# violetamenendez/zest-nerf

Hardware: AMD Instinct MI355X
Metric: rendered rays/sec (1024-ray x 128-sample batch per GPU) (higher is better)
Workload: dtype bf16; 1 GPU; nsff_static_1024x128; rays_per_gpu=1024, samples_per_ray=128, rays_total=1024, collective=none, ranks=1, backend=none

## Files before the change

### zest-nerf_amd/csrc/fused.cuh

```cuda
#pragma once
#include "mlp_engine.cuh"
#include "zest_sample_ops.cuh"

namespace zest {

constexpr int kMaxViews = 16;
constexpr int kCamStride = 24;

struct FusedNet {
    const float *bias;
    const uint4 *tiles;
    const float4 *vol;
    const float4 *imgs;
    const float *w2cs, *intr;
    int D, Hv, Wv, V, H, W;
    int head, v2;
};

struct FusedArgs {
    const float *ndc, *pts, *z, *dir;
    int R, S;
    FusedNet st, dy;
    float frame_idx;
    int white_bkgd;
    int bpr;
    float *partials;
    float *out;
    unsigned long long *stamps;
    int ray_ranges;
};

struct RayState {
    float Ts = 1.f, Tb = 1.f, Tf = 1.f;
    float s[5] = {0, 0, 0, 0, 0}, bl[5] = {0, 0, 0, 0, 0}, fg[4] = {0, 0, 0, 0};
    __device__ __forceinline__ void chain(const float *p, bool dyn) {
#pragma unroll
        for (int i = 0; i < 5; i++) s[i] += Ts * p[1 + i];
        Ts *= p[0];
        if (dyn) {
#pragma unroll
            for (int i = 0; i < 5; i++) bl[i] += Tb * p[7 + i];
            Tb *= p[6];
#pragma unroll
            for (int i = 0; i < 4; i++) fg[i] += Tf * p[13 + i];
            Tf *= p[12];
        }
    }
    __device__ __forceinline__ void emit(int white_bkgd, float *__restrict__ out_row) const {
        float4 *o = reinterpret_cast<float4 *>(out_row);
        const float bg = white_bkgd ? 1.0f - s[4] : 0.0f;
        o[0] = make_float4(s[0] + bg, s[1] + bg, s[2] + bg, s[3]);
        o[1] = make_float4(s[4], bl[0], bl[1], bl[2]);
        o[2] = make_float4(bl[3], fg[0], fg[1], fg[2]);
        float zero = 0.f;
        asm volatile("" : "+v"(zero));
        o[3] = make_float4(fg[3], bl[4], zero, zero);
    }
    __device__ __forceinline__ void save(float *c) const {
        c[0] = Ts, c[1] = Tb, c[2] = Tf;
#pragma unroll
        for (int i = 0; i < 5; i++) c[3 + i] = s[i], c[8 + i] = bl[i];
#pragma unroll
        for (int i = 0; i < 4; i++) c[13 + i] = fg[i];
    }
    __device__ __forceinline__ void load(const float *c) {
        Ts = c[0], Tb = c[1], Tf = c[2];
#pragma unroll
        for (int i = 0; i < 5; i++) s[i] = c[3 + i], bl[i] = c[8 + i];
#pragma unroll
        for (int i = 0; i < 4; i++) fg[i] = c[13 + i];
    }
};
constexpr int kCarryFloats = 20;

template <class Rec>
__device__ __forceinline__ void combine_ray(Rec rec, int bpr, bool dyn, int white_bkgd, float *__restrict__ out_row) {
    RayState st;
    for (int b = 0; b < bpr; b++) st.chain(rec(b), dyn);
    st.emit(white_bkgd, out_row);
}

template <int EP, int C, int L, int NK>
__device__ __forceinline__ void encode_pe_operand(const float (&x)[4], int grp, OpArr<NK, ep_parts(EP)> &op) {
    static_assert((L / 2) * C + 1 <= NK * 8 && L % 2 == 0, "position layout");
    const float quarter = (grp & 1) ? 0.25f : 0.0f;
    const float gscale = (grp & 2) ? 2.0f * 0.15915494309189535f : 0.15915494309189535f;
    const float gband = (grp & 2) ? 2.0f : 1.0f;
    float rev[C];
#pragma unroll
    for (int c = 0; c < C; c++) rev[c] = x[c] * gscale;
    const float raw = grp == 0 ? x[0] : (grp == 1 ? x[1] : (grp == 2 ? x[2] : (C > 3 ? x[3] : 0.0f)));
#pragma unroll
    for (int t = 0; t < NK; t++) {
        float v[8];
#pragma unroll
        for (int e = 0; e < 8; e++) {
            const int m = 8 * t + e;
            if (m < (L / 2) * C) {
                if constexpr (EP == ZEST_PREC_F16X3) {
                    float sn, cs;
                    zest_sincos(x[m % C] * (gband * (float)(1 << (2 * (m / C)))), &sn, &cs);
                    v[e] = (grp & 1) ? cs : sn;
                } else {
                    const float r = fmaf(rev[m % C], (float)(1 << (2 * (m / C))), quarter);
                    v[e] = __builtin_amdgcn_sinf(__builtin_amdgcn_fractf(r));
                }
            } else if (m == (L / 2) * C) {
                v[e] = raw;
            } else {
                v[e] = 0.0f;
            }
        }
        store_tile<EP>(v, op, t);
    }
}

__device__ __forceinline__ float4 zest_color_tap_fast(const float4 *__restrict__ img, int H, int W,
                                                      const float *__restrict__ P, float px, float py, float pz) {
    const float4 r0 = *reinterpret_cast<const float4 *>(P), r1 = *reinterpret_cast<const float4 *>(P + 4),
                 r2 = *reinterpret_cast<const float4 *>(P + 8);
    const float qx = fmaf(pz, r0.z, fmaf(py, r0.y, fmaf(px, r0.x, r0.w)));
    const float qy = fmaf(pz, r1.z, fmaf(py, r1.y, fmaf(px, r1.x, r1.w)));
    const float qz = fmaf(pz, r2.z, fmaf(py, r2.y, fmaf(px, r2.x, r2.w)));
    const float rz = __builtin_amdgcn_rcpf(qz);
    float fx = qx * rz, fy = qy * rz;
    const float wm = (float)(W - 1), hm = (float)(H - 1);
    const float mask = (fx > 0.0f && fx < wm && fy > 0.0f && fy < hm) ? 1.0f : 0.0f;
    fx = fminf(fmaxf(fx, 0.0f), wm), fy = fminf(fmaxf(fy, 0.0f), hm);
    const float x0f = floorf(fx), y0f = floorf(fy);
    const float tx = fx - x0f, ty = fy - y0f;
    const int x0 = (int)x0f, y0 = (int)y0f;
    const int i00 = y0 * W + x0, dx = x0 + 1 < W ? 1 : 0, dy = y0 + 1 < H ? W : 0;
    const float4 a = img[i00], b = img[i00 + dx], d = img[i00 + dy], e = img[i00 + dy + dx];
    const float w00 = (1.0f - tx) * (1.0f - ty), w10 = tx * (1.0f - ty), w01 = (1.0f - tx) * ty, w11 = tx * ty;
    float4 o;
    o.x = fmaf(w11, e.x, fmaf(w01, d.x, fmaf(w10, b.x, w00 * a.x)));
    o.y = fmaf(w11, e.y, fmaf(w01, d.y, fmaf(w10, b.y, w00 * a.y)));
    o.z = fmaf(w11, e.z, fmaf(w01, d.z, fmaf(w10, b.z, w00 * a.z)));
    o.w = mask;
    return o;
}

template <int EP, int NK>
__device__ __forceinline__ void encode_feat_operand(const FusedNet &n, const float *cams_lds,
                                                    const float (&ndc)[4], const float (&pw)[3],
                                                    int grp, bool valid, OpArr<NK, ep_parts(EP)> &op) {
    float v[NK * 8];
#pragma unroll
    for (int i = 0; i < NK * 8; i++) v[i] = 0.0f;
    auto view_tap = [&](int view, float *dst) {
        const int vc = view < n.V ? view : n.V - 1;
        const float *cl = cams_lds + vc * kCamStride;
        float4 o;
        if constexpr (EP == ZEST_PREC_F16X3) {
            ZestCam cam;
#pragma unroll
            for (int i = 0; i < 3; i++) {
#pragma unroll
                for (int j = 0; j < 4; j++) cam.r[i][j] = cl[4 * i + j];
#pragma unroll
                for (int j = 0; j < 3; j++) cam.k[i][j] = cl[12 + 3 * i + j];
            }
            o = zest_color_tap(n.imgs + (size_t)vc * n.H * n.W, n.H, n.W, cam, pw[0], pw[1], pw[2]);
        } else {
            o = zest_color_tap_fast(n.imgs + vc * (n.H * n.W), n.H, n.W, cl, pw[0], pw[1], pw[2]);
        }
        const bool on = view < n.V;
        dst[0] = on ? o.x : 0.f, dst[1] = on ? o.y : 0.f, dst[2] = on ? o.z : 0.f, dst[3] = on ? o.w : 0.f;
    };
    const int rv = feat_volume_round(n.V);
    if (valid) {
        float vv[4] = {0.f, 0.f, 0.f, 0.f};
        if (grp < 2) {
            float fx = zest_unnorm(ndc[0], n.Wv), fy = zest_unnorm(ndc[1], n.Hv), fz = zest_unnorm(ndc[2], n.D);
            fx = fminf(fmaxf(fx, -2.0f), (float)n.Wv + 1.0f);
            fy = fminf(fmaxf(fy, -2.0f), (float)n.Hv + 1.0f);
            fz = fminf(fmaxf(fz, -2.0f), (float)n.D + 1.0f);
            const float x0f = floorf(fx), y0f = floorf(fy), z0f = floorf(fz);
            const float tx = fx - x0f, ty = fy - y0f, tz = fz - z0f;
            const int x0 = (int)x0f, y0 = (int)y0f, z0 = (int)z0f;
            float4 tap[8];
            float wgt[8];
#pragma unroll
            for (int c = 0; c < 8; c++) {
                const int dx = c & 1, dy = (c >> 1) & 1, dz = c >> 2;
                const int xi = x0 + dx, yi = y0 + dy, zi = z0 + dz;
                const bool ok = (unsigned)xi < (unsigned)n.Wv && (unsigned)yi < (unsigned)n.Hv &&
                                (unsigned)zi < (unsigned)n.D;
                const int xc = min(max(xi, 0), n.Wv - 1), yc = min(max(yi, 0), n.Hv - 1),
                          zc = min(max(zi, 0), n.D - 1);
                wgt[c] = ok ? (dx ? tx : 1.0f - tx) * (dy ? ty : 1.0f - ty) * (dz ? tz : 1.0f - tz) : 0.0f;
                tap[c] = n.vol[2 * ((yc * n.Wv + xc) * n.D + zc) + grp];
            }
#pragma unroll
            for (int c = 0; c < 8; c++) {
                vv[0] = fmaf(wgt[c], tap[c].x, vv[0]), vv[1] = fmaf(wgt[c], tap[c].y, vv[1]);
                vv[2] = fmaf(wgt[c], tap[c].z, vv[2]), vv[3] = fmaf(wgt[c], tap[c].w, vv[3]);
            }
        }
#pragma unroll
        for (int r = 0; r < 2 * NK; r++) {
            float *dst = v + 8 * (r >> 1) + 4 * (r & 1);
            if (r < rv) {
                view_tap(4 * r + grp, dst);
            } else if (r == rv) {
                if (n.V > 4 * rv) view_tap(grp >= 2 ? 4 * rv + grp - 2 : n.V, dst);
                if (grp < 2) dst[0] = vv[0], dst[1] = vv[1], dst[2] = vv[2], dst[3] = vv[3];
            }
        }
    }
#pragma unroll
    for (int t = 0; t < NK; t++) {
        float w8[8];
#pragma unroll
        for (int e = 0; e < 8; e++) w8[e] = v[8 * t + e];
        store_tile<EP>(w8, op, t);
    }
}

template <bool PROJ>
__device__ __forceinline__ void stage_cams(const FusedNet &n, float *lds) {
    if (!n.w2cs) return;
    const int nv = n.imgs ? n.V : 1;
    for (int i = threadIdx.x; i < nv * kCamStride; i += blockDim.x) {
        const int v = i / kCamStride, k = i % kCamStride;
        float val = 0.0f;
        if constexpr (PROJ) {
            if (k < 12 && n.intr) {
                const int row = k >> 2, col = k & 3;
                const float *K = n.intr + 9 * v + 3 * row, *Rt = n.w2cs + 16 * v + col;
                val = fmaf(K[2], Rt[8], fmaf(K[1], Rt[4], K[0] * Rt[0]));
            } else if (k >= 12) {
                val = n.w2cs[16 * v + (k - 12)];
            }
        } else {
            if (k < 12) val = n.w2cs[16 * v + k];
            else if (k < 21 && n.intr) val = n.intr[9 * v + (k - 12)];
        }
        lds[i] = val;
    }
}

#ifndef ZEST_FUSED_WAVES
#define ZEST_FUSED_WAVES 8
#endif
constexpr int kFusedWaves = ZEST_FUSED_WAVES;
constexpr int kPartialFloats = 20;
constexpr int fused_cb(int EP) { return EP == ZEST_PREC_F16X3 ? 1 : 2; }

struct BlockSamples {
    float x[4], pw[3], zz, dist;
    bool valid;
};

template <int BS>
__device__ __forceinline__ float block_sum(float v) {
    if constexpr (BS == 32) return lower_half_sum(v);
    v += dpp_f<0xB1>(0.f, v);
    v += dpp_f<0x4E>(0.f, v);
    v += dpp_f<0x141>(0.f, v);
    v += dpp_f<0x140>(0.f, v);
    return readlane_f<0>(v);
}
template <int BS>
__device__ __forceinline__ float block_excl_prod(float f, int c, float *total) {
    if constexpr (BS == 32) return lower_half_excl_prod(f, c, total);
    float v = f;
    v *= dpp_f<0x111>(1.f, v);
    v *= dpp_f<0x112>(1.f, v);
    v *= dpp_f<0x114>(1.f, v);
    v *= dpp_f<0x118>(1.f, v);
    *total = readlane_f<15>(v);
    const float ex = dpp_f<0x138>(1.f, v);
    return c == 0 ? 1.0f : ex;
}

#ifndef ZEST_FUSED_WG_PER_CU
#define ZEST_FUSED_WG_PER_CU 1
#endif
template <int EP, int NT_FEAT_S, bool DYN, int NT_FEAT_D, bool V2S = false>
__global__ __launch_bounds__(kFusedWaves * 64, kFusedWaves * ZEST_FUSED_WG_PER_CU / 4) void fused_blocks_kernel(FusedArgs a) {
    constexpr bool MOD_S = NT_FEAT_S > 0, MOD_D = NT_FEAT_D > 0;
    constexpr int NP = ep_parts(EP), CB = fused_cb(EP), BS = 16 * CB;
    if constexpr (EP == ZEST_PREC_F16) engine_fp16_overflow_clamp();
    constexpr int UNITS_S = stream_units(4, NT_FEAT_S, NP, true), UNITS_D = DYN ? stream_units(6, NT_FEAT_D, NP, true) : 0;
    using Ring = RingTiles<kFusedWaves, UNITS_S, UNITS_D>;
    constexpr bool FEATURELESS = !MOD_S && !MOD_D;
    constexpr int PF = (NP == 1 && FEATURELESS) ? kPrefetchLone : kPrefetch;
    constexpr bool CONT = NP == 1 || FEATURELESS;
    constexpr int kStBytes = DYN ? kFusedWaves * 32 * 24 : 0;
    constexpr int kGapBytes = 2 * kSlots * 4;
    __shared__ __attribute__((aligned(16))) char lds[kRingUnits * 1024 + 2 * kMaxViews * kCamStride * 4 +
                                                     kFusedWaves * 32 * 8 + kGapBytes +
                                                     kFusedWaves * kPartialFloats * 4 + kFusedWaves * 32 * 16 +
                                                     kStBytes + 2 * kCarryFloats * 4];
    static_assert(sizeof(lds) <= 163840, "LDS budget of one workgroup per CU");
    float *cams_s = reinterpret_cast<float *>(lds + kRingUnits * 1024), *cams_d = cams_s + kMaxViews * kCamStride;
    float2 *zd_lds = reinterpret_cast<float2 *>(cams_d + kMaxViews * kCamStride);
    constexpr bool PROJ = EP != ZEST_PREC_F16X3;
    stage_cams<PROJ>(a.st, cams_s);
    if (DYN) stage_cams<PROJ>(a.dy, cams_d);
    char *gap = reinterpret_cast<char *>(zd_lds + kFusedWaves * 32);
    float *rec_lds = reinterpret_cast<float *>(gap + kGapBytes);
    float4 *x_lds = reinterpret_cast<float4 *>(rec_lds + kFusedWaves * kPartialFloats);
    float2 *st_lds = reinterpret_cast<float2 *>(x_lds + kFusedWaves * 32);
    float *carry_lds = reinterpret_cast<float *>(reinterpret_cast<char *>(st_lds) + kStBytes);
    __syncthreads();

    const int lane0 = threadIdx.x & 63;
    const int wave = __builtin_amdgcn_readfirstlane(threadIdx.x >> 6);
    const Ring tiles{lds, (gptr_u4)a.st.tiles, (gptr_u4)a.dy.tiles, lane0, lane0 >> 4, wave,
                     (unsigned)(wave * Ring::kPieces * 64 + lane0) * 16u,
                     (unsigned)(uintptr_t)(__attribute__((address_space(3))) char *)lds +
                         (unsigned)wave * Ring::kPieces * 1024u};
    tiles.init_addr();
    tiles.prologue();

    const bool ranges = a.ray_ranges != 0;
    const int n_wg = (int)gridDim.x;
    const int wg = n_wg % 8 == 0 ? (int)(blockIdx.x % 8) * (n_wg / 8) + (int)(blockIdx.x / 8) : (int)blockIdx.x;
    int range_b0, range_nb;
    if (ranges) {
        range_b0 = (int)((long long)wg * a.R / n_wg) * a.bpr;
        range_nb = (int)((long long)(wg + 1) * a.R / n_wg) * a.bpr - range_b0;
    } else {
        const int n_blocks = a.R * a.bpr;
        const int share = ((n_blocks + kFusedWaves - 1) / kFusedWaves + n_wg - 1) / n_wg * kFusedWaves;
        range_b0 = wg * share, range_nb = min(share, n_blocks - range_b0);
    }
    auto block_of = [&](int pass) {
        const int lb = pass * kFusedWaves + wave;
        return __builtin_amdgcn_readfirstlane(lb < range_nb ? range_b0 + lb : -1);
    };
    auto fetch = [&](int g, int cb, int col, BlockSamples &b) {
        const int r = g >= 0 ? g / a.bpr : 0, s = (g >= 0 ? g % a.bpr : 0) * BS + 16 * cb + col;
        b.valid = g >= 0 && s < a.S;
        b.x[0] = b.x[1] = b.x[2] = 0.f, b.x[3] = a.frame_idx;
        b.pw[0] = b.pw[1] = b.pw[2] = 0.f, b.zz = 0.f, b.dist = 0.f;
        const float *dir = a.dir + 3 * r;
        if (b.valid) {
            const size_t m = (size_t)r * a.S + s;
            const float *zr = a.z + (size_t)r * a.S;
            b.x[0] = a.ndc[3 * m], b.x[1] = a.ndc[3 * m + 1], b.x[2] = a.ndc[3 * m + 2];
            if (a.pts) b.pw[0] = a.pts[3 * m], b.pw[1] = a.pts[3 * m + 1], b.pw[2] = a.pts[3 * m + 2];
            b.zz = zr[s];
            const float dnorm = sqrtf(dir[0] * dir[0] + dir[1] * dir[1] + dir[2] * dir[2]);
            b.dist = ((s + 1 < a.S) ? (zr[s + 1] - b.zz) : 1e10f) * dnorm;
        }
    };
    auto join = [](const f32x4 (&t)[CB], int i) {
        if constexpr (CB == 1) {
            return t[0][i];
        } else {
            const auto r = __builtin_amdgcn_permlane16_swap(__float_as_uint(t[0][i]), __float_as_uint(t[CB - 1][i]), false, false);
            return __uint_as_float(r[0]);
        }
    };
#ifdef ZEST_STAMPS
    unsigned long long st_enc = 0, st_eng = 0, st_comp = 0, st_n = 0;
    const unsigned long long st_t0 = __builtin_amdgcn_s_memtime(), st_r0 = __builtin_amdgcn_s_memrealtime();
#define ZEST_STAMP(var) do { const unsigned long long t_ = __builtin_amdgcn_s_memtime(); var += t_ - st_last; st_last = t_; } while (0)
#else
#define ZEST_STAMP(var) do {} while (0)
#endif
    for (int k = 0; k * kFusedWaves < range_nb; k++) {
        const int pass = k;
#ifdef ZEST_STAMPS
        unsigned long long st_last = __builtin_amdgcn_s_memtime();
        st_n++;
#endif
        const int g = block_of(pass);
        if (__builtin_expect(g < 0, 0)) {
            tiles.finish(0, UNITS_S + UNITS_D);
        } else {
        int lane = lane0;
        asm volatile("" : "+v"(lane));
        const int col = lane & 15, grp = lane >> 4, cbs = lane & (BS - 1);
        int unit = 0;
        f32x4 head_s[CB], rgb_s[CB], head_d[CB], rgb_d[CB];
        auto views_of = [&](const FusedNet &n, const float *cams) {
            return [&, cams](OpArr<1, NP> (&views)[CB]) {
                const float *dir = a.dir + 3 * (g >= 0 ? g / a.bpr : 0);
                float dv[4] = {0.f, 0.f, 0.f, 0.f};
                zest_view_dir(dir, n.w2cs ? cams + (PROJ ? 12 : 0) : nullptr, dv);
                encode_pe_operand<EP, 3, 4, 1>(dv, grp, views[0]);
#pragma unroll
                for (int cb = 1; cb < CB; cb++) views[cb] = views[0];
            };
        };
        OpArr<NT_FEAT_S / 2, NP> feat_s[CB];
#pragma unroll
        for (int cb = 0; cb < CB; cb++) {
            BlockSamples b;
            fetch(g, cb, col, b);
            if (grp == 0) {
                zd_lds[wave * 32 + 16 * cb + col] = make_float2(b.zz, b.valid ? b.dist : -1.0f);
                x_lds[wave * 32 + 16 * cb + col] = make_float4(b.x[0], b.x[1], b.x[2], 0.0f);
            }
            if constexpr (MOD_S) encode_feat_operand<EP, NT_FEAT_S / 2>(a.st, cams_s, b.x, b.pw, grp, b.valid, feat_s[cb]);
            if constexpr (DYN && NT_FEAT_S >= 4) __builtin_amdgcn_sched_barrier(0);
        }
        auto pts_static = [&](OpArr<2, NP> (&o)[CB]) __attribute__((always_inline)) {
#pragma unroll
            for (int cb = 0; cb < CB; cb++) {
                int at = wave * 32 + 16 * cb + col;
                asm volatile("" : "+v"(at));
                const float4 xv = x_lds[at];
                const float x4[4] = {xv.x, xv.y, xv.z, 0.0f};
                encode_pe_operand<EP, 3, 10, 2>(x4, grp, o[cb]);
            }
        };
        auto pts_dynamic = [&](OpArr<3, NP> (&o)[CB]) __attribute__((always_inline)) {
#pragma unroll
            for (int cb = 0; cb < CB; cb++) {
                int at = wave * 32 + 16 * cb + col;
                asm volatile("" : "+v"(at));
                const float4 xv = x_lds[at];
                const float x4[4] = {xv.x, xv.y, xv.z, a.frame_idx};
                encode_pe_operand<EP, 4, 10, 3>(x4, grp, o[cb]);
            }
        };
        ZEST_STAMP(st_enc);
        {
            OpArr<2, NP> pts_keep[CB];
            pts_static(pts_keep);
            auto pts_copy = [&](OpArr<2, NP> (&o)[CB]) __attribute__((always_inline)) {
#pragma unroll
                for (int cb = 0; cb < CB; cb++) o[cb] = pts_keep[cb];
            };
            engine_forward<EP, CB, 4, MOD_S, NT_FEAT_S, V2S, true, PF, CONT>(tiles, unit, pts_copy, feat_s,
                                                                             views_of(a.st, cams_s), head_s, rgb_s);
        }
        ZEST_STAMP(st_eng);
        float rec[kPartialFloats];
#pragma unroll
        for (int i = 0; i < kPartialFloats; i++) rec[i] = 0.f;
        float zz, dist, cr, cg, cb, al_s;
        bool valid;
        {
            const float2 zd = zd_lds[wave * 32 + cbs];
            zz = zd.x, dist = fmaxf(zd.y, 0.0f), valid = zd.y >= 0.0f;
            float sg = join(head_s, 0);
            cr = join(rgb_s, 0), cg = join(rgb_s, 1), cb = join(rgb_s, 2);
            if (V2S) {
                cr = zest_sigmoid(cr), cg = zest_sigmoid(cg), cb = zest_sigmoid(cb), sg = fmaxf(sg, 0.f);
            }
            cr = zest_sigmoid(cr), cg = zest_sigmoid(cg), cb = zest_sigmoid(cb);
            al_s = valid ? 1.0f - expf(-fmaxf(sg, 0.f) * dist) : 0.0f;
            float tot;
            const float w = al_s * block_excl_prod<BS>(1.0f - al_s + 1e-10f, cbs, &tot);
            rec[0] = tot;
            rec[1] = block_sum<BS>(w * cr), rec[2] = block_sum<BS>(w * cg), rec[3] = block_sum<BS>(w * cb);
            rec[4] = block_sum<BS>(w * zz), rec[5] = block_sum<BS>(w);
        }
        if (DYN) {
            const float blend_s = zest_sigmoid(join(head_s, 1));
            if (lane < BS) {
                st_lds[(wave * 3 + 0) * 32 + lane] = make_float2(cr, cg);
                st_lds[(wave * 3 + 1) * 32 + lane] = make_float2(cb, al_s);
                st_lds[(wave * 3 + 2) * 32 + lane] = make_float2(blend_s, 0.0f);
            }
            OpArr<NT_FEAT_D / 2, NP> feat_d[CB];
            if constexpr (MOD_D) {
#pragma unroll
                for (int cbi = 0; cbi < CB; cbi++) {
                    BlockSamples b;
                    fetch(g, cbi, col, b);
                    encode_feat_operand<EP, NT_FEAT_D / 2>(a.dy, cams_d, b.x, b.pw, grp, b.valid, feat_d[cbi]);
                }
            }
            ZEST_STAMP(st_comp);
            {
                OpArr<3, NP> pts_keep[CB];
                pts_dynamic(pts_keep);
                auto pts_copy = [&](OpArr<3, NP> (&o)[CB]) __attribute__((always_inline)) {
#pragma unroll
                    for (int cb = 0; cb < CB; cb++) o[cb] = pts_keep[cb];
                };
                engine_forward<EP, CB, 6, MOD_D, NT_FEAT_D, false, true, PF, CONT>(tiles, unit, pts_copy, feat_d,
                                                                                   views_of(a.dy, cams_d), head_d, rgb_d);
            }
            ZEST_STAMP(st_eng);
            const float2 s0 = st_lds[(wave * 3 + 0) * 32 + cbs], s1 = st_lds[(wave * 3 + 1) * 32 + cbs],
                         s2 = st_lds[(wave * 3 + 2) * 32 + cbs];
            cr = s0.x, cg = s0.y, cb = s1.x, al_s = s1.y;
            const float blend = s2.x;
            const float er = zest_sigmoid(join(rgb_d, 0)), eg = zest_sigmoid(join(rgb_d, 1)),
                        eb = zest_sigmoid(join(rgb_d, 2));
            const float sg_d = join(head_d, 0);
            const float a_fg = valid ? 1.0f - expf(-fmaxf(sg_d, 0.f) * dist) : 0.0f;
            const float a_d = a_fg * blend, a_st = al_s * (1.0f - blend);
            float tot_b, tot_f;
            const float Tb = block_excl_prod<BS>((1.0f - a_d) * (1.0f - a_st) + 1e-10f, cbs, &tot_b);
            const float wf = a_fg * block_excl_prod<BS>(1.0f - a_fg + 1e-10f, cbs, &tot_f);
            const float wd = Tb * a_d, ws = Tb * a_st;
            rec[6] = tot_b;
            rec[7] = block_sum<BS>(wd * er + ws * cr), rec[8] = block_sum<BS>(wd * eg + ws * cg);
            rec[9] = block_sum<BS>(wd * eb + ws * cb), rec[10] = block_sum<BS>((wd + ws) * zz);
            rec[11] = block_sum<BS>(wd);
            rec[12] = tot_f;
            rec[13] = block_sum<BS>(wf * er), rec[14] = block_sum<BS>(wf * eg), rec[15] = block_sum<BS>(wf * eb);
            rec[16] = block_sum<BS>(wf * zz);
        }
        if (lane == 0 && g >= 0) {
            float4 *o = ranges ? reinterpret_cast<float4 *>(rec_lds + wave * kPartialFloats)
                               : reinterpret_cast<float4 *>(a.partials + (size_t)g * kPartialFloats);
#pragma unroll
            for (int i = 0; i < (DYN ? 5 : 2); i++)
                o[i] = make_float4(rec[4 * i], rec[4 * i + 1], rec[4 * i + 2], rec[4 * i + 3]);
        }
        }
        if (ranges) {
            __syncthreads();
            const int rb = g >= 0 ? g % a.bpr : 0;
            if (lane0 == 0 && g >= 0 && (wave == 0 || rb == 0)) {
                RayState st;
                if (rb != 0) st.load(carry_lds + ((k + 1) & 1) * kCarryFloats);
                const int n = min(a.bpr - rb, kFusedWaves - wave);
                for (int b = 0; b < n; b++) st.chain(rec_lds + (wave + b) * kPartialFloats, DYN);
                if (rb + n == a.bpr) st.emit(a.white_bkgd, a.out + (size_t)(g / a.bpr) * 16);
                else st.save(carry_lds + (k & 1) * kCarryFloats);
            }
        }
        ZEST_STAMP(st_comp);
    }
    tiles.drain();
#ifdef ZEST_STAMPS
    if (a.stamps && lane0 == 0) {
        unsigned long long *o = a.stamps + (size_t)(blockIdx.x * kFusedWaves + wave) * 8;
        o[0] = __builtin_amdgcn_s_memtime() - st_t0, o[1] = st_enc, o[2] = st_eng, o[3] = st_comp;
        o[4] = tiles.t_wait, o[5] = tiles.t_issue, o[6] = __builtin_amdgcn_s_memrealtime() - st_r0,
        o[7] = st_n | (tiles.t_vm << 16);
    }
#endif
}

#define ZEST_FUSED_VARIANT(ptag, EP, tag, NTS, DYN, NTD, V2S) ZEST_FUSED_VARIANT_(ptag, EP, tag, NTS, DYN, NTD, V2S)
#define ZEST_FUSED_VARIANT_(ptag, EP, tag, NTS, DYN, NTD, V2S)                                   \
    int fused_launch_##ptag##_##tag(const FusedArgs &a, int blocks, hipStream_t stream) {        \
        hipLaunchKernelGGL((fused_blocks_kernel<EP, NTS, DYN, NTD, V2S>), dim3(blocks),          \
                           dim3(kFusedWaves * 64), 0, stream, a);                                \
        ZEST_RETURN_LAUNCH("zest_render_fused_fwd(" #ptag "_" #tag ")");                         \
    }                                                                                            \
    int fused_units_##ptag##_##tag(int which) {                                                  \
        return which == 0 ? stream_units(4, NTS, ep_parts(EP), true) : (DYN ? stream_units(6, NTD, ep_parts(EP), true) : 0); \
    }

#define ZEST_FUSED_DECL1(ptag, tag)                                                     \
    int fused_launch_##ptag##_##tag(const FusedArgs &a, int blocks, hipStream_t stream); \
    int fused_units_##ptag##_##tag(int which);
#define ZEST_FUSED_DECL(tag) ZEST_FUSED_DECL1(bf16, tag) ZEST_FUSED_DECL1(f16, tag) ZEST_FUSED_DECL1(x3, tag)
ZEST_FUSED_DECL(s0)
ZEST_FUSED_DECL(s2)
ZEST_FUSED_DECL(s4)
ZEST_FUSED_DECL(s0d0)
ZEST_FUSED_DECL(s2d0)
ZEST_FUSED_DECL(s4d0)
ZEST_FUSED_DECL(s2d2)
ZEST_FUSED_DECL(s4d2)
ZEST_FUSED_DECL(s2v)
ZEST_FUSED_DECL(s4v)

}
```

### zest-nerf_amd/csrc/fused.hip

```cpp
#include <string.h>
#include "fused.cuh"
#include "mlp_plan.h"

namespace zest {

__global__ void fused_combine_kernel(const float *__restrict__ partials, int R, int bpr, int dyn,
                                     int white_bkgd, float *__restrict__ out) {
    const int r = blockIdx.x * blockDim.x + threadIdx.x;
    if (r >= R) return;
    combine_ray([&](int b) { return partials + ((size_t)r * bpr + b) * kPartialFloats; }, bpr, dyn != 0,
                white_bkgd, out + (size_t)r * 16);
}

}

namespace {

bool fill_net(const zest_mlp_desc *d, const void *packed, const zest_view_set *vs, int pts_ch, int precision,
              zest::FusedNet *n, int *nt_feat, int *units, const char **err) {
    memset(n, 0, sizeof(*n));
    if (!d || !packed) return *err = "descriptor and packed weights are required", false;
    if (d->in_ch_pts != pts_ch) return *err = "unexpected in_ch_pts for this slot", false;
    if (d->net_type != 0 && d->net_type != 2) return *err = "net_type must be 0 ('v0') or 2 ('v2')", false;
    zest::MlpPlan plan;
    if (!zest::build_plan(*d, precision, zest::ORDER_ACC, &plan, err, false, true)) return false;
    n->bias = (const float *)((const char *)packed + plan.stream_off);
    n->tiles = (const uint4 *)((const char *)n->bias + plan.bias_bytes);
    n->head = d->head, n->v2 = d->net_type == 2;
    *nt_feat = d->use_feat ? plan.nt_feat : 0;
    *units = plan.n_tiles;
    if (((uintptr_t)packed & 15) != 0) return *err = "packed weights must be 16-byte aligned", false;
    if (vs) {
        n->w2cs = vs->w2cs, n->intr = vs->intrinsics;
        n->vol = (const float4 *)vs->vol_cl, n->imgs = (const float4 *)vs->imgs_cl;
        n->D = vs->D, n->Hv = vs->Hv, n->Wv = vs->Wv, n->V = vs->V, n->H = vs->H, n->W = vs->W;
    }
    if (d->use_feat) {
        if (!vs || !vs->vol_cl || !vs->imgs_cl || !vs->w2cs || !vs->intrinsics)
            return *err = "a net with features needs volume, images and cameras", false;
        if (vs->D < 1 || vs->Hv < 1 || vs->Wv < 1 || vs->H < 2 || vs->W < 2)
            return *err = "bad volume / image shape", false;
        if ((long long)vs->D * vs->Hv * vs->Wv >= (1LL << 30))
            return *err = "volume too large for the fused kernel's 32-bit voxel indices (2^30 voxels)", false;
        if (vs->V < 1 || vs->V > zest::kMaxViews || 8 + 4 * vs->V != d->in_ch_feat)
            return *err = "view count does not match in_ch_feat = 8 + 4V", false;
        if (((uintptr_t)vs->vol_cl | (uintptr_t)vs->imgs_cl) & 15)
            return *err = "volume / images must be 16-byte aligned", false;
    } else {
        n->vol = nullptr, n->imgs = nullptr;
    }
    return true;
}

}

#ifdef ZEST_STAMPS
constexpr size_t kStampBytes = 1024 * 8 * 8 * 8;
#else
constexpr size_t kStampBytes = 0;
#endif

static int g_pass_shape = 0;

extern "C" int zest_render_fused_set_passes(int shape) {
    ZEST_CHECK_ARG(shape >= 0 && shape <= 2,
                   "zest_render_fused_set_passes: shape must be 0 (auto), 1 (dense: equal block shares) or 2 (ray ranges)");
    g_pass_shape = shape;
    return 0;
}

extern "C" int zest_render_fused_pass_shape(int R, int S, int precision, int cus, int *ray_ranges, int *n_wg,
                                            int *rounds) {
    ZEST_CHECK_ARG(R >= 0 && S >= 1 && zest::prec_is_engine(precision) && ray_ranges,
                   "zest_render_fused_pass_shape: bad argument");
    if (cus <= 0) {
        int dev = 0;
        if (hipGetDevice(&dev) != hipSuccess ||
            hipDeviceGetAttribute(&cus, hipDeviceAttributeMultiprocessorCount, dev) != hipSuccess)
            cus = 256;
    }
    const int bs = 16 * zest::fused_cb(precision), bpr = (S + bs - 1) / bs;
    const int W = zest::kFusedWaves;
    const int P = zest_div_up((long long)R * bpr, W), G0 = P < cus ? P : cus;
    const int dense_rounds = G0 ? zest_div_up(P, G0) : 0, dense_wg = G0 ? zest_div_up(P, dense_rounds) : 0;
    const int n = R < cus ? R : cus;
    const int range_rounds = n ? zest_div_up((long long)zest_div_up(R, n) * bpr, W) : 0;
    int take = range_rounds <= dense_rounds ? 1 : 0;
    if (g_pass_shape == 1) take = 0;
    if (g_pass_shape == 2) take = 1;
    *ray_ranges = take;
    if (n_wg) *n_wg = take ? n : dense_wg;
    if (rounds) *rounds = take ? range_rounds : dense_rounds;
    return 0;
}

extern "C" size_t zest_render_fused_workspace(int R, int S) {
    if (R <= 0 || S <= 0) return 16 + kStampBytes;
    return (size_t)R * ((S + 15) / 16) * zest::kPartialFloats * sizeof(float) + kStampBytes;
}

extern "C" int zest_render_fused_fwd(const float *ndc, const float *pts, const float *z,
                                     const float *rays_dir, int R, int S,
                                     const zest_mlp_desc *desc_static, const void *packed_static,
                                     const zest_view_set *views_static,
                                     const zest_mlp_desc *desc_dynamic, const void *packed_dynamic,
                                     const zest_view_set *views_dynamic, float frame_idx,
                                     int precision, int white_bkgd, void *workspace, float *out,
                                     void *stream) {
    if (R == 0) return 0;
    ZEST_CHECK_ARG(ndc && z && rays_dir && out && workspace,
                   "zest_render_fused_fwd: ndc, z, rays_dir, workspace, out required");
    ZEST_CHECK_ARG(((uintptr_t)workspace & 15) == 0, "zest_render_fused_fwd: workspace must be 16-byte aligned");
    ZEST_CHECK_ARG(R >= 0 && S >= 1, "zest_render_fused_fwd: bad shape R=%d S=%d", R, S);
    ZEST_CHECK_ARG(zest::prec_is_engine(precision),
                   "zest_render_fused_fwd: precision must be ZEST_PREC_BF16, _F16 or _F16X3 (the exact-product "
                   "fp32 kernel exists per operator only: zest_mlp_fwd)");
    ZEST_CHECK_ARG(((uintptr_t)out & 15) == 0, "zest_render_fused_fwd: out must be 16-byte aligned");
    zest::FusedArgs a;
    memset(&a, 0, sizeof(a));
    a.ndc = ndc, a.pts = pts, a.z = z, a.dir = rays_dir, a.R = R, a.S = S;
    a.frame_idx = frame_idx, a.white_bkgd = white_bkgd, a.out = out;
    const int bs = 16 * zest::fused_cb(precision);
    a.bpr = (S + bs - 1) / bs, a.partials = (float *)workspace;
#ifdef ZEST_STAMPS
    a.stamps = (unsigned long long *)((char *)workspace + zest_render_fused_workspace(R, S) - kStampBytes);
#endif
    const char *err = nullptr;
    int nts = 0, ntd = 0, units_s = 0, units_d = 0;
    ZEST_CHECK_ARG(fill_net(desc_static, packed_static, views_static, 63, precision, &a.st, &nts, &units_s, &err),
                   "zest_render_fused_fwd: static net: %s", err);
    const bool dyn = desc_dynamic != nullptr;
    if (dyn) {
        ZEST_CHECK_ARG(fill_net(desc_dynamic, packed_dynamic, views_dynamic, 84, precision, &a.dy, &ntd, &units_d, &err),
                       "zest_render_fused_fwd: dynamic net: %s", err);
        ZEST_CHECK_ARG(desc_static->head == ZEST_HEAD_BLEND && desc_dynamic->head == ZEST_HEAD_DYNAMIC,
                       "zest_render_fused_fwd: blending needs a static net with the blend head and "
                       "a dynamic net with the scene-flow heads");
    }
    ZEST_CHECK_ARG(pts || (!a.st.vol && !a.dy.vol), "zest_render_fused_fwd: pts required with features");
    if (R == 0) return 0;
    int dev = 0, cus = 256;
    if (hipGetDevice(&dev) != hipSuccess ||
        hipDeviceGetAttribute(&cus, hipDeviceAttributeMultiprocessorCount, dev) != hipSuccess)
        cus = 256;
    int blocks = 0;
    zest_render_fused_pass_shape(R, S, precision, cus, &a.ray_ranges, &blocks, nullptr);
    hipStream_t st = (hipStream_t)stream;
    const bool v2s = a.st.v2 != 0;
    ZEST_CHECK_ARG(!(v2s && (dyn || nts == 0)),
                   "zest_render_fused_fwd: a 'v2' net is rendered by the single-net kernels with features only");
    const int key = (v2s ? 1000 : 0) + (dyn ? 100 : 0) + nts * 10 + ntd;
    int rc = -1;
#define ZEST_CASE1(ptag, tag)                                                                    \
    ZEST_CHECK_ARG(zest::fused_units_##ptag##_##tag(0) == units_s && zest::fused_units_##ptag##_##tag(1) == units_d, \
                   "zest_render_fused_fwd: packed stream is %d+%d units, kernel expects %d+%d",  \
                   units_s, units_d, zest::fused_units_##ptag##_##tag(0), zest::fused_units_##ptag##_##tag(1)); \
    rc = zest::fused_launch_##ptag##_##tag(a, blocks, st);
#define ZEST_CASE(k, tag)                                                                        \
    case k:                                                                                      \
        if (precision == ZEST_PREC_BF16) { ZEST_CASE1(bf16, tag) }                               \
        else if (precision == ZEST_PREC_F16) { ZEST_CASE1(f16, tag) }                            \
        else { ZEST_CASE1(x3, tag) }                                                             \
        break;
    switch (key) {
        ZEST_CASE(0, s0)
        ZEST_CASE(20, s2)
        ZEST_CASE(40, s4)
        ZEST_CASE(100, s0d0)
        ZEST_CASE(120, s2d0)
        ZEST_CASE(140, s4d0)
        ZEST_CASE(122, s2d2)
        ZEST_CASE(142, s4d2)
        ZEST_CASE(1020, s2v)
        ZEST_CASE(1040, s4v)
        default:
            zest_set_error("zest_render_fused_fwd: no fused variant for %d static / %d dynamic feature "
                           "tiles%s", nts, ntd, dyn ? "" : " (static only)");
            return (int)hipErrorInvalidValue;
    }
#undef ZEST_CASE
#undef ZEST_CASE1
    if (rc != 0 || a.ray_ranges) return rc;
    hipLaunchKernelGGL(zest::fused_combine_kernel, dim3(zest_div_up(R, 128)), dim3(128), 0, st,
                       a.partials, R, a.bpr, dyn ? 1 : 0, white_bkgd, out);
    ZEST_RETURN_LAUNCH("zest_render_fused_fwd(combine)");
}
```

### zest-nerf_amd/csrc/mlp.hip

```cpp
#include <string.h>
#include <map>
#include <mutex>
#include <tuple>
#include "mlp_plan.h"
#include "zest_common.cuh"
#include "mlp_engine.cuh"

namespace {

using zest::MlpPlan;

struct DevPlan {
    MlpPlan plan;
    uint32_t *tile_src = nullptr, *bias_src = nullptr, *hdr_src = nullptr;
    uint8_t *unit_part = nullptr;
};

std::mutex g_mu;
std::map<std::tuple<int, int, int, int, int, int, int, int, int, int, int, int>, DevPlan *> g_plans;

constexpr int kOrderBwd = 99;
constexpr int kOrderFold = 98;

DevPlan *get_plan(const zest_mlp_desc &d, int precision, int order, bool need_tables) {
    int dev = 0;
    if (hipGetDevice(&dev) != hipSuccess) dev = 0;
    std::lock_guard<std::mutex> lk(g_mu);
    auto key = std::make_tuple(d.in_ch_pts, d.use_feat ? d.in_ch_feat : 0, d.in_ch_views,
                               d.use_feat, d.net_type, d.head, precision, order, d.depth, d.width, d.skip_mask, dev);
    auto it = g_plans.find(key);
    DevPlan *dp = it == g_plans.end() ? nullptr : it->second;
    if (!dp) {
        dp = new DevPlan();
        const char *err = nullptr;
        const bool ok = order == kOrderBwd    ? zest::build_bwd_plan(d, &dp->plan, &err)
                        : order == kOrderFold ? zest::build_plan(d, precision, zest::ORDER_ACC, &dp->plan, &err, true, true)
                                              : zest::build_plan(d, precision, order, &dp->plan, &err);
        if (!ok) {
            zest_set_error("MLP shape not supported: %s", err);
            delete dp;
            return nullptr;
        }
        g_plans[key] = dp;
    }
    if (need_tables && !dp->tile_src) {
        const size_t nt = dp->plan.tile_src.size() * 4, nb = dp->plan.bias_src.size() * 4;
        const size_t nh = dp->plan.hdr_src.size() * 4, np = dp->plan.unit_part.size();
        hipError_t e = hipMalloc(&dp->tile_src, nt);
        if (e == hipSuccess) e = hipMalloc(&dp->unit_part, np ? np : 4);
        if (e == hipSuccess && np) e = hipMemcpy(dp->unit_part, dp->plan.unit_part.data(), np, hipMemcpyHostToDevice);
        if (e == hipSuccess) e = hipMalloc(&dp->bias_src, nb ? nb : 4);
        if (e == hipSuccess) e = hipMalloc(&dp->hdr_src, nh ? nh : 4);
        if (e == hipSuccess) e = hipMemcpy(dp->tile_src, dp->plan.tile_src.data(), nt, hipMemcpyHostToDevice);
        if (e == hipSuccess && nb) e = hipMemcpy(dp->bias_src, dp->plan.bias_src.data(), nb, hipMemcpyHostToDevice);
        if (e == hipSuccess && nh) e = hipMemcpy(dp->hdr_src, dp->plan.hdr_src.data(), nh, hipMemcpyHostToDevice);
        if (e != hipSuccess) {
            zest_set_error("zest_mlp_pack: uploading gather tables: %s", hipGetErrorString(e));
            dp->tile_src = nullptr;
            return nullptr;
        }
    }
    return dp;
}

inline int order_for(int precision) {
    return zest::prec_is_engine(precision) ? zest::ORDER_ACC : zest::ORDER_NATURAL;
}

struct ParamTable {
    const float *p[2 * zest::kParamSlots];
};

__global__ __launch_bounds__(zest::kW) void fold_view_kernel(const float *__restrict__ wv, const float *__restrict__ bv,
                                                             const float *__restrict__ wf, const float *__restrict__ bf,
                                                             int ld_v, float *__restrict__ wc, float *__restrict__ bc) {
    constexpr int W = zest::kW;
    const int r = blockIdx.x, c = threadIdx.x;
    if (r < W / 2) {
        double acc = 0.0;
        for (int k = 0; k < W; k++) acc += (double)wv[(size_t)r * ld_v + k] * (double)wf[(size_t)k * W + c];
        wc[(size_t)r * W + c] = (float)acc;
    } else if (c < W / 2) {
        double acc = 0.0;
        for (int k = 0; k < W; k++) acc += (double)wv[(size_t)c * ld_v + k] * (double)bf[k];
        bc[c] = (float)(acc + (double)bv[c]);
    } else {
        bc[c] = 0.0f;
    }
}
static_assert(zest::kFoldScratchBytes == zest::kFoldBiasOffset + (size_t)zest::kW * 4, "bc [W/2] and W/2 floats of padding");

template <int PREC>
__global__ void pack_kernel(ParamTable pt, const uint32_t *__restrict__ tile_src, size_t n_w,
                            const uint32_t *__restrict__ bias_src, size_t n_b,
                            const uint8_t *__restrict__ unit_part,
                            float *__restrict__ bias_out, void *__restrict__ w_out) {
    const size_t i = (size_t)blockIdx.x * blockDim.x + threadIdx.x;
    if (i < n_b) {
        const uint32_t s = bias_src[i];
        bias_out[i] = s == 0xFFFFFFFFu ? 0.0f : pt.p[2 * (s >> 24) + 1][s & 0xFFFFFF];
    }
    if (i < n_w) {
        const uint32_t s = tile_src[i];
        const float v = s == 0xFFFFFFFFu ? 0.0f : pt.p[2 * (s >> 24)][s & 0xFFFFFF];
        if (PREC == ZEST_PREC_BF16) {
            ((__hip_bfloat16 *)w_out)[i] = __float2bfloat16(v);
        } else if (PREC == ZEST_PREC_F16) {
            ((_Float16 *)w_out)[i] = (_Float16)v;
        } else if (PREC == ZEST_PREC_F16X3) {
            const _Float16 hi = (_Float16)v;
            ((_Float16 *)w_out)[i] = unit_part[i / 512] ? (_Float16)((v - (float)hi) * 2048.0f) : hi;
        } else {
            ((float *)w_out)[i] = v;
        }
    }
}

__global__ void pack_headers_kernel(ParamTable pt, const uint32_t *__restrict__ hdr_src, size_t n,
                                    char *__restrict__ w_out) {
    const size_t i = (size_t)blockIdx.x * blockDim.x + threadIdx.x;
    if (i >= n) return;
    const uint32_t s = hdr_src[i];
    if (s == 0xFFFFFFFFu) return;
    const size_t unit = i / 64, j = i % 64;
    ((float *)(w_out + unit * 1024))[j] = pt.p[2 * (s >> 24) + 1][s & 0xFFFFFF];
}

struct F32Op {
    int njb, nseg, kind0, nt0, kind1, nt1, mod, relu, tile_base, tiles_per_jb, bias_block;
    int src_h, dst;
};
struct F32Prog {
    F32Op op[zest::kNumOps];
    int n_ops, W;
    int P, F, Vw, C_in, C_out, nt_feat, net_v2, act_out, head;
    int rows_pts, rows_feat;
};

constexpr int kF32Samples = 32;

__global__ __launch_bounds__(256, 1) void mlp_f32_kernel(F32Prog pr, const float *__restrict__ bias,
                                                         const float4 *__restrict__ tiles,
                                                         const float *__restrict__ x, int M,
                                                         float *__restrict__ out) {
    extern __shared__ __attribute__((aligned(16))) float smem[];
    float *b_pts = smem;
    float *b_feat = b_pts + pr.rows_pts * 32;
    float *b_views = b_feat + pr.rows_feat * 32;
    float *b_h[2] = {b_views + 32 * 32, b_views + 32 * 32 + pr.W * 32};
    const int tid = threadIdx.x, lane = tid & 63, wave = tid >> 6;
    const int col = lane & 31, half = lane >> 5;
    const int n_in_rows = pr.rows_pts + pr.rows_feat + 32;

    for (int m0 = blockIdx.x * kF32Samples; m0 < M; m0 += gridDim.x * kF32Samples) {
        __syncthreads();
        for (int i = tid; i < n_in_rows * 32; i += 256) smem[i] = 0.0f;
        __syncthreads();
        const int nvalid = min(kF32Samples, M - m0);
        for (int i = tid; i < nvalid * pr.C_in; i += 256) {
            const int s = i / pr.C_in, c = i % pr.C_in;
            const float v = x[(size_t)m0 * pr.C_in + i];
            float *dst = c < pr.P ? b_pts + c * 32
                                  : (c < pr.P + pr.F ? b_feat + (c - pr.P) * 32
                                                     : b_views + (c - pr.P - pr.F) * 32);
            dst[s] = v;
        }
        __syncthreads();
#pragma unroll 1
        for (int o = 0; o < pr.n_ops; o++) {
            const F32Op op = pr.op[o];
            for (int jb = wave; jb < op.njb; jb += 4) {
                const float4 *tp = tiles + ((size_t)op.tile_base + (size_t)jb * op.tiles_per_jb) * 64 + lane;
                f32x16 acc, macc;
                {
                    const float *bb = bias + (size_t)(op.bias_block + jb) * 32 + half * 16;
#pragma unroll
                    for (int i = 0; i < 16; i++) acc[i] = bb[i];
                }
                if (op.mod) {
                    const float *mb = bias + (size_t)jb * 32 + half * 16;
#pragma unroll
                    for (int i = 0; i < 16; i++) macc[i] = mb[i];
                    for (int t = 0; t < pr.nt_feat; t++, tp += 64) {
                        const float4 a = *tp;
                        const float *bp = b_feat + (t * 8 + 4 * half) * 32 + col;
                        macc = __builtin_amdgcn_mfma_f32_32x32x2f32(a.x, bp[0], macc, 0, 0, 0);
                        macc = __builtin_amdgcn_mfma_f32_32x32x2f32(a.y, bp[32], macc, 0, 0, 0);
                        macc = __builtin_amdgcn_mfma_f32_32x32x2f32(a.z, bp[64], macc, 0, 0, 0);
                        macc = __builtin_amdgcn_mfma_f32_32x32x2f32(a.w, bp[96], macc, 0, 0, 0);
                    }
                }
                for (int sg = 0; sg < op.nseg; sg++) {
                    const int kind = sg ? op.kind1 : op.kind0, nt = sg ? op.nt1 : op.nt0;
                    const float *src = kind == zest::SEG_PTS ? b_pts
                                       : kind == zest::SEG_VIEWS ? b_views : b_h[op.src_h];
                    for (int t = 0; t < nt; t++, tp += 64) {
                        const float4 a = *tp;
                        const float *bp = src + (t * 8 + 4 * half) * 32 + col;
                        acc = __builtin_amdgcn_mfma_f32_32x32x2f32(a.x, bp[0], acc, 0, 0, 0);
                        acc = __builtin_amdgcn_mfma_f32_32x32x2f32(a.y, bp[32], acc, 0, 0, 0);
                        acc = __builtin_amdgcn_mfma_f32_32x32x2f32(a.z, bp[64], acc, 0, 0, 0);
                        acc = __builtin_amdgcn_mfma_f32_32x32x2f32(a.w, bp[96], acc, 0, 0, 0);
                    }
                }
#pragma unroll
                for (int i = 0; i < 16; i++) {
                    const int row = 32 * jb + (i & 3) + 8 * (i >> 2) + 4 * half;
                    float v = acc[i];
                    if (op.mod) v = pr.net_v2 ? v + macc[i] : v * macc[i];
                    if (op.relu) v = fmaxf(v, 0.0f);
                    if (op.dst < 2) {
                        b_h[op.dst][row * 32 + col] = v;
                    } else if (col < nvalid) {
                        float *orow = out + (size_t)(m0 + col) * pr.C_out;
                        if (o == pr.n_ops - 1) {
                            if (row < 3) orow[row] = pr.act_out ? zest_sigmoid(v) : v;
                        } else if (row == 0) {
                            orow[3] = pr.act_out ? fmaxf(v, 0.0f) : v;
                        } else if (3 + row < pr.C_out) {
                            const bool is_sf = pr.head == ZEST_HEAD_DYNAMIC && row <= 6;
                            orow[3 + row] = is_sf ? tanhf(v) : zest_sigmoid(v);
                        }
                    }
                }
            }
            __syncthreads();
        }
    }
}

F32Prog make_f32_prog(const MlpPlan &p) {
    F32Prog pr = {};
    const int D = p.shape.D, t = (D - 1) & 1;
    pr.n_ops = p.n_ops, pr.W = p.shape.W;
    for (int o = 0; o < p.n_ops; o++) {
        const zest::OpPlan &s = p.op[o];
        F32Op &d = pr.op[o];
        const int src_h = o < D ? (o + 1) & 1 : (o == D + 2 ? 1 - t : t);
        const int dst = o < D ? o & 1 : (o == D + 1 ? 1 - t : (o == D + 2 ? t : 2));
        d.njb = s.njb, d.nseg = s.nseg, d.kind0 = s.seg[0].kind, d.nt0 = s.seg[0].ntiles;
        d.kind1 = s.seg[1].kind, d.nt1 = s.seg[1].ntiles, d.mod = s.mod, d.relu = s.relu;
        d.tile_base = s.tile_base, d.tiles_per_jb = s.tiles_per_jb, d.bias_block = s.bias_block;
        d.src_h = src_h, d.dst = dst;
    }
    pr.P = p.desc.in_ch_pts, pr.F = p.desc.use_feat ? p.desc.in_ch_feat : 0, pr.Vw = p.desc.in_ch_views;
    pr.C_in = pr.P + pr.F + pr.Vw;
    pr.C_out = p.desc.head == ZEST_HEAD_NONE ? 4 : (p.desc.head == ZEST_HEAD_BLEND ? 5 : 12);
    pr.nt_feat = p.nt_feat, pr.net_v2 = p.desc.net_type >= 2, pr.act_out = p.desc.net_type == 2, pr.head = p.desc.head;
    pr.rows_pts = p.nt_pts * 8, pr.rows_feat = p.nt_feat * 8;
    return pr;
}

}

namespace zest {
size_t bwd_stream_bytes(const zest_mlp_desc &d) {
    DevPlan *dp = get_plan(d, ZEST_PREC_BF16, kOrderBwd, false);
    return dp ? dp->plan.bytes : 0;
}
int bwd_stream_units_of(const zest_mlp_desc &d) {
    DevPlan *dp = get_plan(d, ZEST_PREC_BF16, kOrderBwd, false);
    return dp ? dp->plan.tail_unit0 : -1;
}
int pack_bwd_stream(const zest_mlp_desc &d, const float *const *params, void *packed, hipStream_t stream) {
    DevPlan *dp = get_plan(d, ZEST_PREC_BF16, kOrderBwd, true);
    if (!dp) return (int)hipErrorInvalidValue;
    const MlpPlan &p = dp->plan;
    ParamTable pt = {};
    for (int i = 0; i < 2 * ZEST_P_COUNT; i++) pt.p[i] = params[i];
    const size_t n_w = p.tile_src.size(), n_h = p.hdr_src.size();
    hipLaunchKernelGGL(pack_kernel<ZEST_PREC_BF16>, dim3(zest_div_up(n_w, 256)), dim3(256), 0, stream, pt, dp->tile_src,
                       n_w, dp->bias_src, (size_t)0, dp->unit_part, (float *)packed, packed);
    hipLaunchKernelGGL(pack_headers_kernel, dim3(zest_div_up(n_h, 256)), dim3(256), 0, stream, pt, dp->hdr_src, n_h,
                       (char *)packed);
    ZEST_RETURN_LAUNCH("zest_mlp_train16_pack");
}
}

extern "C" size_t zest_mlp_packed_bytes(const zest_mlp_desc *desc, int precision) {
    if (!desc) return 0;
    if (zest::prec_is_engine(precision)) {
        DevPlan *df = get_plan(*desc, precision, kOrderFold, false);
        return df ? df->plan.stream_off + df->plan.bytes : 0;
    }
    DevPlan *dp = get_plan(*desc, precision, order_for(precision), false);
    return dp ? dp->plan.bytes : 0;
}

extern "C" int zest_mlp_pack(const zest_mlp_desc *desc, int precision, const float *const *params,
                             void *packed, void *stream) {
    ZEST_CHECK_ARG(desc && params && packed, "zest_mlp_pack: null argument");
    DevPlan *dp = get_plan(*desc, precision, order_for(precision), true);
    if (!dp) return (int)hipErrorInvalidValue;
    const MlpPlan &p = dp->plan;
    DevPlan *df = zest::prec_is_engine(precision) ? get_plan(*desc, precision, kOrderFold, true) : nullptr;
    if (zest::prec_is_engine(precision) && !df) return (int)hipErrorInvalidValue;
    ParamTable pt = {};
    for (int i = 0; i < 2 * ZEST_P_COUNT; i++) pt.p[i] = params[i];
    bool need[ZEST_P_COUNT] = {};
    for (int i = 0; i < p.shape.D; i++) need[i] = true;
    need[ZEST_P_PTS_BIAS] = desc->use_feat != 0;
    need[ZEST_P_VIEWS] = need[ZEST_P_FEATURE] = need[ZEST_P_ALPHA] = need[ZEST_P_RGB] = true;
    need[ZEST_P_HEAD0] = desc->head != ZEST_HEAD_NONE;
    need[ZEST_P_HEAD1] = desc->head == ZEST_HEAD_DYNAMIC;
    for (int i = 0; i < ZEST_P_COUNT; i++)
        ZEST_CHECK_ARG(!need[i] || (params[2 * i] && params[2 * i + 1]),
                       "zest_mlp_pack: parameter slot %d (weight and bias) is required", i);
    ZEST_CHECK_ARG(((uintptr_t)packed & 15) == 0, "zest_mlp_pack: packed must be 16-byte aligned");
    auto pack_stream = [&](const DevPlan *q, char *base) {
        const size_t n_w = q->plan.tile_src.size(), n_b = q->plan.bias_src.size();
        const size_t n = n_w > n_b ? n_w : n_b;
        void *w_out = base + q->plan.bias_bytes;
#define ZEST_PACK(PREC)                                                                            \
    hipLaunchKernelGGL(pack_kernel<PREC>, dim3(zest_div_up(n, 256)), dim3(256), 0, (hipStream_t)stream, \
                       pt, q->tile_src, n_w, q->bias_src, n_b, q->unit_part, (float *)base, w_out)
        if (zest::prec_is_engine(precision)) {
            if (precision == ZEST_PREC_BF16) ZEST_PACK(ZEST_PREC_BF16);
            else if (precision == ZEST_PREC_F16) ZEST_PACK(ZEST_PREC_F16);
            else ZEST_PACK(ZEST_PREC_F16X3);
            const size_t n_h = q->plan.hdr_src.size();
            if (n_h)
                hipLaunchKernelGGL(pack_headers_kernel, dim3(zest_div_up(n_h, 256)), dim3(256), 0,
                                   (hipStream_t)stream, pt, q->hdr_src, n_h, (char *)w_out);
        } else {
            ZEST_PACK(ZEST_PREC_F32);
        }
#undef ZEST_PACK
    };
    pack_stream(dp, (char *)packed);
    if (df) {
        float *wc = (float *)((char *)packed + zest::fold_scratch_offset(p.bytes));
        float *bc = (float *)((char *)wc + zest::kFoldBiasOffset);
        hipLaunchKernelGGL(fold_view_kernel, dim3(zest::kW / 2 + 1), dim3(zest::kW), 0, (hipStream_t)stream,
                           params[2 * ZEST_P_VIEWS], params[2 * ZEST_P_VIEWS + 1], params[2 * ZEST_P_FEATURE],
                           params[2 * ZEST_P_FEATURE + 1], zest::kW + desc->in_ch_views, wc, bc);
        pt.p[2 * zest::kFoldSlot] = wc, pt.p[2 * zest::kFoldSlot + 1] = bc;
        pack_stream(df, (char *)packed + df->plan.stream_off);
    }
    ZEST_RETURN_LAUNCH("zest_mlp_pack");
}

extern "C" int zest_mlp_fwd(const zest_mlp_desc *desc, int precision, const void *packed,
                            const float *x, int M, float *out, void *stream) {
    if (M == 0) return 0;
    ZEST_CHECK_ARG(desc && packed && x && out, "zest_mlp_fwd: null argument");
    ZEST_CHECK_ARG(M >= 0, "zest_mlp_fwd: M=%d", M);
    DevPlan *dp = get_plan(*desc, precision, zest::prec_is_engine(precision) ? kOrderFold : order_for(precision), false);
    if (!dp) return (int)hipErrorInvalidValue;
    if (M == 0) return 0;
    const MlpPlan &p = dp->plan;
    const float *bias = (const float *)((const char *)packed + p.stream_off);
    const void *tiles = (const char *)bias + p.bias_bytes;
    if (precision == ZEST_PREC_F32) {
        const F32Prog pr = make_f32_prog(p);
        const size_t lds = (size_t)(pr.rows_pts + pr.rows_feat + 32 + 2 * pr.W) * 32 * sizeof(float);
        const int blocks = zest_div_up(M, kF32Samples);
        hipLaunchKernelGGL(mlp_f32_kernel, dim3(blocks < 4096 ? blocks : 4096), dim3(256), lds,
                           (hipStream_t)stream, pr, bias, (const float4 *)tiles, x, M, out);
        ZEST_RETURN_LAUNCH("zest_mlp_fwd(f32)");
    }
    return zest::mlp_engine_launch(p, tiles, x, M, out, (hipStream_t)stream);
}
```

### zest-nerf_amd/csrc/mlp_engine.cuh

```cuda
#pragma once
#include <hip/hip_bf16.h>
#include "mlp_plan.h"
#include "zest_common.cuh"

typedef __attribute__((ext_vector_type(16))) float f32x16;
typedef __attribute__((ext_vector_type(4))) float f32x4;
typedef __attribute__((ext_vector_type(8))) short bf16x8;
typedef __attribute__((ext_vector_type(4))) float v4f;
typedef __attribute__((ext_vector_type(4))) unsigned v4u;
typedef const __attribute__((address_space(1))) v4u *gptr_u4;

namespace zest {

constexpr int stream_units_raw(int nt_pts, int nt_feat, int parts = 1, bool fold = false) {
    const int mod = nt_feat * parts, P = nt_pts * parts, H = 16 * parts;
    return 8 * (1 + mod + P) + 6 * 8 * (1 + mod + H) + 8 * (1 + mod + P + H)
           + (1 + H) + (fold ? 0 : 8 * (1 + H)) + 4 * (1 + H + 2 * parts) + (1 + H / 2);
}
constexpr int stream_units(int nt_pts, int nt_feat, int parts = 1, bool fold = false) {
    return (stream_units_raw(nt_pts, nt_feat, parts, fold) + kStreamAlign - 1) / kStreamAlign * kStreamAlign;
}
static_assert(stream_units_raw(4, 0) == 1262 && stream_units_raw(4, 0, 1, true) == 1126 &&
              stream_units(4, 0, 1, true) == 9 * kStreamAlign, "unit counts of the headline net (DESIGN.md 3.1)");

#ifndef ZEST_CHUNK
#define ZEST_CHUNK 16
#define ZEST_SLOTS 8
#define ZEST_AHEAD 4
#endif
constexpr int kChunk = ZEST_CHUNK, kSlots = ZEST_SLOTS, kRingUnits = kChunk * kSlots, kAhead = ZEST_AHEAD;
static_assert(kStreamAlign % kRingUnits == 0, "stream padding must be a multiple of the ring size");
static_assert(kSlots >= kAhead + 1, "a slot is refilled while the previous chunk may still be read");

#ifndef ZEST_ISSUERS
#define ZEST_ISSUERS 8
#endif
template <int NW, int UNITS_A, int UNITS_B>
struct RingTiles {
    static constexpr int kIssuers = ZEST_ISSUERS < NW ? ZEST_ISSUERS : NW;
    static constexpr int kPieces = kChunk / kIssuers;
    static constexpr int kChunksA = UNITS_A / kChunk, kChunks = (UNITS_A + UNITS_B) / kChunk;
    static_assert(kChunk % kIssuers == 0 && UNITS_A % kRingUnits == 0 && UNITS_B % kRingUnits == 0, "");
    char *ring;
    gptr_u4 src_a, src_b;
    int lane, grp, wave;
    unsigned voff;
    unsigned lds_wave_base;
#ifdef ZEST_STAMPS
    mutable unsigned long long t_wait = 0, t_issue = 0, t_vm = 0;
#endif

    __device__ __forceinline__ void issue(int chunk) const {
        if (kIssuers < NW && wave >= kIssuers) return;
        const int c = chunk % kChunks;
        unsigned off = (unsigned)((c < kChunksA ? c : c - kChunksA) * kChunk * 1024);
        asm volatile("" : "+s"(off));
        const __attribute__((address_space(1))) char *sb =
            (const __attribute__((address_space(1))) char *)(c < kChunksA ? src_a : src_b) + off;
        const unsigned dst = lds_wave_base + (c % kSlots) * kChunk * 1024;
        static_assert(kPieces == 1 || kPieces == 2 || kPieces == 4, "pieces per wave");
        if (kPieces == 1)
            asm volatile("s_mov_b32 m0, %2\n\ts_nop 0\n\tglobal_load_lds_dwordx4 %0, %1"
                         :: "v"(voff), "s"(sb), "s"(dst) : "memory", "m0");
        else if (kPieces == 2)
            asm volatile("s_mov_b32 m0, %2\n\ts_nop 0\n\tglobal_load_lds_dwordx4 %0, %1\n\t"
                         "global_load_lds_dwordx4 %0, %1 offset:1024"
                         :: "v"(voff), "s"(sb), "s"(dst) : "memory", "m0");
        else
            asm volatile("s_mov_b32 m0, %2\n\ts_nop 0\n\tglobal_load_lds_dwordx4 %0, %1\n\t"
                         "global_load_lds_dwordx4 %0, %1 offset:1024\n\t"
                         "global_load_lds_dwordx4 %0, %1 offset:2048\n\t"
                         "global_load_lds_dwordx4 %0, %1 offset:3072"
                         :: "v"(voff), "s"(sb), "s"(dst) : "memory", "m0");
    }
    __device__ __forceinline__ void prologue() const {
#pragma unroll
        for (int c = 0; c < kAhead; c++) issue(c);
    }
    __device__ __forceinline__ void enter_chunk(int chunk) const {
#ifdef ZEST_STAMPS
        const unsigned long long t0 = __builtin_amdgcn_s_memtime();
#endif
        asm volatile("s_waitcnt vmcnt(%0)" ::"i"((kAhead - 1) * kPieces) : "memory");
#ifdef ZEST_STAMPS
        t_vm += __builtin_amdgcn_s_memtime() - t0;
#endif
        __builtin_amdgcn_s_barrier();
        asm volatile("" ::: "memory");
#ifdef ZEST_STAMPS
        const unsigned long long t1 = __builtin_amdgcn_s_memtime();
#endif
        issue(chunk + kAhead);
#ifdef ZEST_STAMPS
        t_wait += t1 - t0, t_issue += __builtin_amdgcn_s_memtime() - t1;
#endif
    }
    __device__ __forceinline__ void touch(int unit) const {
        if (unit % kChunk == 0) enter_chunk(unit / kChunk);
    }
    mutable unsigned rd_lo = 0, rd_hi = 0, rb_lo = 0, rb_hi = 0;
    __device__ __forceinline__ void init_addr() const {
        const unsigned base = (unsigned)(uintptr_t)(__attribute__((address_space(3))) char *)ring;
        rd_lo = base + lane * 16, rd_hi = rd_lo + 65536, rb_lo = base + grp * 16, rb_hi = rb_lo + 65536;
        asm volatile("" : "+v"(rd_lo), "+v"(rd_hi), "+v"(rb_lo), "+v"(rb_hi));
    }
    static_assert(kRingUnits <= 128, "two 64 KiB windows");
    template <class T>
    static __device__ __forceinline__ const __attribute__((address_space(3))) T *lds_at(unsigned addr) {
        return (const __attribute__((address_space(3))) T *)(uintptr_t)addr;
    }
    __device__ __forceinline__ bf16x8 load(int unit) const {
        touch(unit);
        const int r = unit % kRingUnits;
        const v4u v = *lds_at<v4u>((r < 64 ? rd_lo : rd_hi) + (r % 64) * 1024);
        return *reinterpret_cast<const bf16x8 *>(&v);
    }
    __device__ __forceinline__ f32x4 load_bias(int unit, int which, int rt) const {
        if (which == 0 && rt == 0) touch(unit);
        const int r = unit % kRingUnits;
        return *lds_at<v4f>((r < 64 ? rb_lo : rb_hi) + (r % 64) * 1024 + which * 128 + rt * 64);
    }
    __device__ __forceinline__ void finish(int unit, int end) const {
#pragma unroll
        for (int u = (unit + kChunk - 1) / kChunk * kChunk; u < end; u += kChunk) enter_chunk(u / kChunk);
    }
    __device__ __forceinline__ void drain() const { asm volatile("s_waitcnt vmcnt(0)" ::: "memory"); }
};

constexpr int ep_parts(int EP) { return EP == ZEST_PREC_F16X3 ? 2 : 1; }
constexpr float kLoScale = 2048.0f, kLoUnscale = 1.0f / 2048.0f;

typedef __attribute__((ext_vector_type(2))) float f32x2_t;
typedef __attribute__((ext_vector_type(2))) __bf16 bf16x2_t;
typedef __attribute__((ext_vector_type(2))) _Float16 f16x2_t;
typedef __attribute__((ext_vector_type(8))) _Float16 f16x8_t;

template <int EP>
__device__ __forceinline__ unsigned pack_pair(float lo, float hi) {
    const f32x2_t f = {lo, hi};
    if constexpr (EP == ZEST_PREC_BF16) {
        const bf16x2_t r = __builtin_convertvector(f, bf16x2_t);
        return __builtin_bit_cast(unsigned, r);
    } else {
        const f16x2_t r = __builtin_convertvector(f, f16x2_t);
        return __builtin_bit_cast(unsigned, r);
    }
}
__device__ __forceinline__ unsigned pack_bf16(float lo, float hi) { return pack_pair<ZEST_PREC_BF16>(lo, hi); }
__device__ __forceinline__ unsigned short bf16_bits(float v) { return (unsigned short)(pack_bf16(v, 0.f) & 0xFFFFu); }

__device__ __forceinline__ void split_pair(float a, float b, unsigned &hi, unsigned &lo) {
    const f32x2_t f = {a, b};
    const f16x2_t h = __builtin_convertvector(f, f16x2_t);
    const f32x2_t back = __builtin_convertvector(h, f32x2_t);
    const f32x2_t rem = {(a - back[0]) * kLoScale, (b - back[1]) * kLoScale};
    const f16x2_t l = __builtin_convertvector(rem, f16x2_t);
    hi = __builtin_bit_cast(unsigned, h), lo = __builtin_bit_cast(unsigned, l);
}

template <int EP>
__device__ __forceinline__ f32x4 mfma16(bf16x8 a, bf16x8 b, f32x4 c) {
    if constexpr (EP == ZEST_PREC_BF16)
        return __builtin_amdgcn_mfma_f32_16x16x32_bf16(a, b, c, 0, 0, 0);
    else
        return __builtin_amdgcn_mfma_f32_16x16x32_f16(__builtin_bit_cast(f16x8_t, a), __builtin_bit_cast(f16x8_t, b),
                                                      c, 0, 0, 0);
}

template <int EP>
__device__ __forceinline__ float relu1(float v) {
    return __builtin_amdgcn_fmed3f(v, 0.0f, EP == ZEST_PREC_BF16 ? 3.0e38f : 65504.0f);
}

template <int N, int NP = 1>
struct OpArr {
    bf16x8 t[NP][N > 0 ? N : 1];
};

template <int EP, int N>
__device__ __forceinline__ void store_tile(const float (&v)[8], OpArr<N, ep_parts(EP)> &op, int k) {
    if constexpr (EP == ZEST_PREC_F16X3) {
        uint4 h, l;
        split_pair(v[0], v[1], h.x, l.x), split_pair(v[2], v[3], h.y, l.y);
        split_pair(v[4], v[5], h.z, l.z), split_pair(v[6], v[7], h.w, l.w);
        op.t[0][k] = __builtin_bit_cast(bf16x8, h), op.t[1][k] = __builtin_bit_cast(bf16x8, l);
    } else {
        const uint4 q = make_uint4(pack_pair<EP>(v[0], v[1]), pack_pair<EP>(v[2], v[3]), pack_pair<EP>(v[4], v[5]),
                                   pack_pair<EP>(v[6], v[7]));
        op.t[0][k] = __builtin_bit_cast(bf16x8, q);
    }
}

typedef __attribute__((ext_vector_type(2))) short s16x2_t;
__device__ __forceinline__ unsigned relu_bf16x2(unsigned u) {
    const s16x2_t r = __builtin_elementwise_max(__builtin_bit_cast(s16x2_t, u), s16x2_t{0, 0});
    return __builtin_bit_cast(unsigned, r);
}
template <int EP, int N>
__device__ __forceinline__ void store_tile_relu16(const float (&v)[8], OpArr<N, 1> &op, int k) {
    const uint4 q = make_uint4(relu_bf16x2(pack_pair<EP>(v[0], v[1])), relu_bf16x2(pack_pair<EP>(v[2], v[3])),
                               relu_bf16x2(pack_pair<EP>(v[4], v[5])), relu_bf16x2(pack_pair<EP>(v[6], v[7])));
    op.t[0][k] = __builtin_bit_cast(bf16x8, q);
}
__device__ __forceinline__ void engine_fp16_overflow_clamp() {
    __builtin_amdgcn_s_setreg((0 << 11) | (23 << 6) | 1, 1);
}

#ifdef ZEST_PREFETCH
constexpr int kPrefetch = ZEST_PREFETCH, kPrefetchLone = ZEST_PREFETCH;
#else
constexpr int kPrefetch = 3, kPrefetchLone = 6;
#endif

template <int NP, int PF>
struct RowBlockPre {
    f32x4 bias[2], mbias[2];
    bf16x8 win[PF][NP];
};

struct NoSink {
    __device__ __forceinline__ void operator()(int, int, int, const float (&)[8]) const {}
};

template <int EP, int CB, int NJB, int NKA, int NKB, bool MOD, int NKF, bool RELU, int MODE, bool V2, int PF, bool CONT,
          class Tiles, class Sink = NoSink>
__device__ __forceinline__ void engine_layer(const Tiles &tiles, int &unit,
                                             const OpArr<NKA, ep_parts(EP)> (&opa)[CB],
                                             const OpArr<NKB, ep_parts(EP)> (&opb)[CB],
                                             const OpArr<NKF, ep_parts(EP)> (&opf)[CB],
                                             OpArr<8, ep_parts(EP)> (&out)[CB], f32x4 (&keep)[CB],
                                             int sink_id = 0, const Sink &sink = Sink()) {
    constexpr int NP = ep_parts(EP);
    constexpr bool X3 = EP == ZEST_PREC_F16X3;
    constexpr int NM = MOD ? 2 * NKF : 0, T = NM + 2 * (NKA + NKB);
    static_assert(T >= 1, "empty layer");
    constexpr bool kPackedRelu = RELU && MODE == 0 && EP != ZEST_PREC_F16X3 && __is_same(Sink, NoSink);
    constexpr int P = PF < T ? PF : T;
    auto preload_header = [&](RowBlockPre<NP, PF> &p, int u0) {
#pragma unroll
        for (int rt = 0; rt < 2; rt++) {
            p.bias[rt] = tiles.load_bias(u0, 0, rt);
            if (MOD) p.mbias[rt] = tiles.load_bias(u0, 1, rt);
        }
    };
    auto preload_tile = [&](RowBlockPre<NP, PF> &p, int u0, int k) {
#pragma unroll
        for (int pt = 0; pt < NP; pt++) p.win[k][pt] = tiles.load(u0 + 1 + NP * k + pt);
    };
    auto preload = [&](RowBlockPre<NP, PF> &p, int u0) {
        preload_header(p, u0);
#pragma unroll
        for (int k = 0; k < P; k++) preload_tile(p, u0, k);
    };
    RowBlockPre<NP, PF> pre;
    preload(pre, unit);
#pragma unroll
    for (int jb = 0; jb < NJB; jb++) {
        const int u0 = unit;
        f32x4 acc[2][CB], macc[2][CB], corr[2][CB], mcorr[2][CB];
        bf16x8 win[P][NP];
#pragma unroll
        for (int k = 0; k < P; k++)
#pragma unroll
            for (int pt = 0; pt < NP; pt++) win[k][pt] = pre.win[k][pt];
#pragma unroll
        for (int rt = 0; rt < 2; rt++)
#pragma unroll
            for (int cb = 0; cb < CB; cb++) {
                acc[rt][cb] = pre.bias[rt];
                if (MOD) macc[rt][cb] = pre.mbias[rt];
                if (X3) corr[rt][cb] = f32x4{0.f, 0.f, 0.f, 0.f}, mcorr[rt][cb] = f32x4{0.f, 0.f, 0.f, 0.f};
            }
#pragma unroll
        for (int k = 0; k < T; k++) {
            bf16x8 a[NP];
#pragma unroll
            for (int pt = 0; pt < NP; pt++) a[pt] = win[k % P][pt];
            const int rt = k % 2, kt = (k < NM ? k : k - NM) / 2;
#pragma unroll
            for (int cb = 0; cb < CB; cb++) {
                auto opnd = [&](int pt) -> bf16x8 {
                    if (k < NM) return opf[cb].t[pt][k < NM ? kt : 0];
                    if (kt < NKA) return opa[cb].t[pt][(k >= NM && kt < NKA) ? kt : 0];
                    return opb[cb].t[pt][(k >= NM && kt >= NKA) ? kt - NKA : 0];
                };
                if (k < NM) {
                    macc[rt][cb] = mfma16<EP>(a[0], opnd(0), macc[rt][cb]);
                    if constexpr (X3) {
                        mcorr[rt][cb] = mfma16<EP>(a[0], opnd(NP - 1), mcorr[rt][cb]);
                        mcorr[rt][cb] = mfma16<EP>(a[NP - 1], opnd(0), mcorr[rt][cb]);
                    }
                } else {
                    acc[rt][cb] = mfma16<EP>(a[0], opnd(0), acc[rt][cb]);
                    if constexpr (X3) {
                        corr[rt][cb] = mfma16<EP>(a[0], opnd(NP - 1), corr[rt][cb]);
                        corr[rt][cb] = mfma16<EP>(a[NP - 1], opnd(0), corr[rt][cb]);
                    }
                }
            }
            if (k + P < T) {
#pragma unroll
                for (int pt = 0; pt < NP; pt++) win[k % P][pt] = tiles.load(u0 + 1 + NP * (k + P) + pt);
            } else if (CONT && jb + 1 < NJB) {
                if (k + P == T) preload_header(pre, u0 + 1 + NP * T);
                preload_tile(pre, u0 + 1 + NP * T, k + P - T);
            }
        }
        unit = u0 + 1 + NP * T;
        if (!CONT && jb + 1 < NJB) preload(pre, unit);
#pragma unroll
        for (int cb = 0; cb < CB; cb++) {
            float v[8];
#pragma unroll
            for (int i = 0; i < 8; i++) {
                v[i] = acc[i >> 2][cb][i & 3];
                if (X3) v[i] = fmaf(corr[i >> 2][cb][i & 3], kLoUnscale, v[i]);
            }
            if (MOD) {
                float mv[8];
#pragma unroll
                for (int i = 0; i < 8; i++) {
                    mv[i] = macc[i >> 2][cb][i & 3];
                    if (X3) mv[i] = fmaf(mcorr[i >> 2][cb][i & 3], kLoUnscale, mv[i]);
                }
#pragma unroll
                for (int i = 0; i < 8; i++) v[i] = V2 ? v[i] + mv[i] : v[i] * mv[i];
            }
            if (RELU && !kPackedRelu) {
#pragma unroll
                for (int i = 0; i < 8; i++) v[i] = relu1<EP>(v[i]);
            }
            if (MODE == 0) {
                if constexpr (kPackedRelu) store_tile_relu16<EP>(v, out[cb], jb);
                else store_tile<EP>(v, out[cb], jb);
                sink(sink_id, jb, cb, v);
            } else if (jb == 0) {
                keep[cb] = f32x4{v[0], v[1], v[2], v[3]};
            }
        }
    }
}

template <int EP, int CB, int NU_PTS, bool MOD, int NU_FEAT, bool V2, bool FOLD = false, int PF = kPrefetch,
          bool CONT = false, class Tiles, class PtsFn, class ViewsFn, class Sink = NoSink>
__device__ __forceinline__ void engine_forward(const Tiles &tiles, int &unit, PtsFn pts_fn,
                                               const OpArr<NU_FEAT / 2, ep_parts(EP)> (&feat)[CB], ViewsFn views_fn,
                                               f32x4 (&head)[CB], f32x4 (&rgb)[CB], const Sink &sink = Sink()) {
    constexpr int KP = NU_PTS / 2, KF = NU_FEAT / 2, NP = ep_parts(EP);
    static_assert(NU_PTS % 2 == 0 && NU_FEAT % 2 == 0, "units per row block come in row-tile pairs");
    OpArr<8, NP> hA[CB], hB[CB];
    OpArr<0, NP> none[CB];
    f32x4 unused[CB];
    const int unit0 = unit;
    {
        OpArr<KP, NP> pts[CB];
        pts_fn(pts);
        engine_layer<EP, CB, 8, KP, 0, MOD, KF, true, 0, V2, PF, CONT>(tiles, unit, pts, none, feat, hA, unused, 0, sink);
    }
    engine_layer<EP, CB, 8, 8, 0, MOD, KF, true, 0, V2, PF, CONT>(tiles, unit, hA, none, feat, hB, unused, 1, sink);
    engine_layer<EP, CB, 8, 8, 0, MOD, KF, true, 0, V2, PF, CONT>(tiles, unit, hB, none, feat, hA, unused, 2, sink);
    engine_layer<EP, CB, 8, 8, 0, MOD, KF, true, 0, V2, PF, CONT>(tiles, unit, hA, none, feat, hB, unused, 3, sink);
    engine_layer<EP, CB, 8, 8, 0, MOD, KF, true, 0, V2, PF, CONT>(tiles, unit, hB, none, feat, hA, unused, 4, sink);
    {
        OpArr<KP, NP> pts[CB];
        pts_fn(pts);
        engine_layer<EP, CB, 8, KP, 8, MOD, KF, true, 0, V2, PF, CONT>(tiles, unit, pts, hA, feat, hB, unused, 5, sink);
    }
    engine_layer<EP, CB, 8, 8, 0, MOD, KF, true, 0, V2, PF, CONT>(tiles, unit, hB, none, feat, hA, unused, 6, sink);
    engine_layer<EP, CB, 8, 8, 0, MOD, KF, true, 0, V2, PF, CONT>(tiles, unit, hA, none, feat, hB, unused, 7, sink);
    engine_layer<EP, CB, 1, 8, 0, false, KF, false, 1, V2, PF, CONT>(tiles, unit, hB, none, feat, hA, head);
    if constexpr (!FOLD)
        engine_layer<EP, CB, 8, 8, 0, false, KF, false, 0, V2, PF, CONT>(tiles, unit, hB, none, feat, hA, unused, 8, sink);
    OpArr<8, NP> (&vin)[CB] = FOLD ? hB : hA, (&vout)[CB] = FOLD ? hA : hB;
    OpArr<1, NP> views[CB];
    views_fn(views);
    engine_layer<EP, CB, 4, 8, 1, false, KF, true, 0, V2, PF, CONT>(tiles, unit, vin, views, feat, vout, unused, 9, sink);
    OpArr<4, NP> h128[CB];
#pragma unroll
    for (int cb = 0; cb < CB; cb++)
#pragma unroll
        for (int pt = 0; pt < NP; pt++)
#pragma unroll
            for (int k = 0; k < 4; k++) h128[cb].t[pt][k] = vout[cb].t[pt][k];
    engine_layer<EP, CB, 1, 4, 0, false, KF, false, 1, V2, PF, CONT>(tiles, unit, h128, none, feat, vin, rgb);
    tiles.finish(unit, unit0 + stream_units(NU_PTS, MOD ? NU_FEAT : 0, NP, FOLD));
    unit = unit0 + stream_units(NU_PTS, MOD ? NU_FEAT : 0, NP, FOLD);
}

int mlp_engine_launch(const MlpPlan &p, const void *tiles, const float *x, int M, float *out,
                    hipStream_t stream);

}
```

### zest-nerf_amd/csrc/mlp_engine.hip

```cpp
#include "mlp_engine.cuh"
#include "mlp_train16.h"
#include "mlp_operands.cuh"

namespace zest {

constexpr int kMlpWaves = 8;
constexpr int mlp_cb(int EP) { return EP == ZEST_PREC_F16X3 ? 1 : 2; }

__device__ __forceinline__ void stash_store(uint4 *p, uint4 q) {
    __builtin_nontemporal_store(__builtin_bit_cast(v4u, q), reinterpret_cast<v4u *>(p));
}

template <int CB>
struct StashSink {
    uint4 *tiles;
    uint2 *masks;
    long long block;
    int lane;
    mutable unsigned lo[CB], hi[CB];
    __device__ __forceinline__ void operator()(int id, int jb, int cb, const float (&v)[8]) const {
        const int t = id < 8 ? 8 * id + jb : (id == 8 ? 64 + jb : 72 + jb);
        uint4 q = make_uint4(pack_bf16(v[0], v[1]), pack_bf16(v[2], v[3]), pack_bf16(v[4], v[5]), pack_bf16(v[6], v[7]));
        stash_store(&tiles[((block * kStashTiles + t) * CB + cb) * 64 + lane], q);
        if (id == 8) return;
        unsigned bits = 0;
#pragma unroll
        for (int i = 0; i < 8; i++) bits |= (v[i] > 0.0f ? 1u : 0u) << i;
        if (jb == 0) lo[cb] = 0, hi[cb] = 0;
        if (jb < 4) lo[cb] |= bits << (8 * jb);
        else hi[cb] |= bits << (8 * (jb - 4));
        const int last = id == 9 ? 3 : 7, mid = id == 9 ? 8 : id;
        if (jb == last) masks[((block * kStashMasks + mid) * CB + cb) * 64 + lane] = make_uint2(lo[cb], hi[cb]);
    }
};

template <int EP, int NT_PTS, bool MOD, int NT_FEAT, bool TRAIN = false, bool V2 = false>
__global__ __launch_bounds__(kMlpWaves * 64, kMlpWaves / 4) void mlp_engine_kernel(
    const uint4 *__restrict__ tiles_g, const float *__restrict__ x, int M, int P, int F, int C_in, int C_out, int head,
    int act_out, float *__restrict__ out, uint4 *__restrict__ stash_tiles = nullptr, uint2 *__restrict__ stash_masks = nullptr) {
    constexpr bool FOLD = !TRAIN;
    constexpr int NP = ep_parts(EP), CB = mlp_cb(EP), UNITS = stream_units(NT_PTS, MOD ? NT_FEAT : 0, NP, FOLD);
    using Ring = RingTiles<kMlpWaves, UNITS, 0>;
    if constexpr (EP == ZEST_PREC_F16) engine_fp16_overflow_clamp();
    __shared__ __attribute__((aligned(16))) char lds[kRingUnits * 1024 + 2 * kSlots * 4];
    const int lane = threadIdx.x & 63, col = lane & 15, grp = lane >> 4;
    const int wave = __builtin_amdgcn_readfirstlane(threadIdx.x >> 6);
    const Ring tiles{lds, (gptr_u4)tiles_g, (gptr_u4)tiles_g, lane, grp, wave,
                     (unsigned)(wave * Ring::kPieces * 64 + lane) * 16u,
                     (unsigned)(uintptr_t)(__attribute__((address_space(3))) char *)lds +
                         (unsigned)wave * Ring::kPieces * 1024u};
    tiles.init_addr();
    tiles.prologue();
    const int n_blocks = (M + 16 * CB - 1) / (16 * CB), n_pass = (n_blocks + kMlpWaves - 1) / kMlpWaves;
    for (int pass = blockIdx.x; pass < n_pass; pass += gridDim.x) {
        const long long m_base = ((long long)pass * kMlpWaves + wave) * (16 * CB);
        OpArr<NT_PTS / 2, NP> pts[CB];
        OpArr<NT_FEAT / 2, NP> feat[CB];
#pragma unroll
        for (int cb = 0; cb < CB; cb++) {
            const long long m = m_base + 16 * cb + col;
            const bool valid = m < M;
            const float *xrow = x + (size_t)(valid ? m : 0) * C_in;
            load_pe_operand<EP, NT_PTS == 4 ? 3 : 4, 10, NT_PTS / 2>(xrow, valid, grp, pts[cb]);
            if (MOD) load_feat_operand<EP, NT_FEAT / 2>(xrow + P, F, valid, grp, feat[cb]);
            if constexpr (TRAIN) {
                uint4 *st = stash_tiles + (((long long)pass * kMlpWaves + wave) * kStashTiles * CB + cb) * 64 + lane;
#pragma unroll
                for (int k = 0; k < NT_PTS / 2; k++) stash_store(&st[(size_t)(kStashPts + k) * CB * 64], __builtin_bit_cast(uint4, pts[cb].t[0][k]));
                if (MOD) {
#pragma unroll
                    for (int k = 0; k < NT_FEAT / 2; k++) stash_store(&st[(size_t)(kStashFeat + k) * CB * 64], __builtin_bit_cast(uint4, feat[cb].t[0][k]));
                }
            }
        }
        auto views_fn = [&](OpArr<1, NP> (&views)[CB]) {
#pragma unroll
            for (int cb = 0; cb < CB; cb++) {
                const long long m = m_base + 16 * cb + col;
                const bool valid = m < M;
                load_pe_operand<EP, 3, 4, 1>(x + (size_t)(valid ? m : 0) * C_in + P + F, valid, grp, views[cb]);
                if constexpr (TRAIN)
                    stash_store(&stash_tiles[((((long long)pass * kMlpWaves + wave) * kStashTiles + kStashViews) * CB + cb) * 64 + lane],
                                __builtin_bit_cast(uint4, views[cb].t[0][0]));
            }
        };
        f32x4 headt[CB], rgbt[CB];
        int unit = 0;
        auto pts_fn = [&](OpArr<NT_PTS / 2, NP> (&o)[CB]) {
#pragma unroll
            for (int cb = 0; cb < CB; cb++) o[cb] = pts[cb];
        };
        if constexpr (TRAIN) {
            const StashSink<CB> sink{stash_tiles, stash_masks, (long long)pass * kMlpWaves + wave, lane, {}, {}};
            engine_forward<EP, CB, NT_PTS, MOD, NT_FEAT, V2, false>(tiles, unit, pts_fn, feat, views_fn, headt, rgbt, sink);
        } else {
            engine_forward<EP, CB, NT_PTS, MOD, NT_FEAT, V2, true>(tiles, unit, pts_fn, feat, views_fn, headt, rgbt);
        }
#pragma unroll
        for (int cb = 0; cb < CB; cb++) {
            const long long m = m_base + 16 * cb + col;
            if (m >= M) continue;
            float *o = out + (size_t)m * C_out;
            if (grp == 0) {
                o[0] = act_out ? zest_sigmoid(rgbt[cb][0]) : rgbt[cb][0];
                o[1] = act_out ? zest_sigmoid(rgbt[cb][1]) : rgbt[cb][1];
                o[2] = act_out ? zest_sigmoid(rgbt[cb][2]) : rgbt[cb][2];
                o[3] = act_out ? fmaxf(headt[cb][0], 0.0f) : headt[cb][0];
                if (head == ZEST_HEAD_BLEND) o[4] = zest_sigmoid(headt[cb][1]);
                if (head == ZEST_HEAD_DYNAMIC)
                    o[4] = tanhf(headt[cb][1]), o[5] = tanhf(headt[cb][2]), o[6] = tanhf(headt[cb][3]);
            } else if (head == ZEST_HEAD_DYNAMIC && grp == 1) {
                o[7] = tanhf(headt[cb][0]), o[8] = tanhf(headt[cb][1]), o[9] = tanhf(headt[cb][2]);
                o[10] = zest_sigmoid(headt[cb][3]);
            } else if (head == ZEST_HEAD_DYNAMIC && grp == 2) {
                o[11] = zest_sigmoid(headt[cb][0]);
            }
        }
    }
    tiles.drain();
}

template <int EP, int NT_PTS, bool MOD, int NT_FEAT, bool TRAIN = false, bool V2 = false>
static int launch_one(const MlpPlan &p, const void *tiles, const float *x, int M,
                      float *out, hipStream_t stream, void *stash_tiles = nullptr, void *stash_masks = nullptr) {
    constexpr int units = stream_units(NT_PTS, MOD ? NT_FEAT : 0, ep_parts(EP), !TRAIN);
    if (p.n_tiles != units || (p.fold != 0) != !TRAIN) {
        zest_set_error("zest_mlp_fwd(engine): plan has %d stream units (fold %d), kernel expects %d (fold %d)", p.n_tiles,
                       p.fold, units, TRAIN ? 0 : 1);
        return (int)hipErrorInvalidValue;
    }
    const zest_mlp_desc &d = p.desc;
    const int F = d.use_feat ? d.in_ch_feat : 0;
    const int C_in = d.in_ch_pts + F + d.in_ch_views;
    const int C_out = d.head == ZEST_HEAD_NONE ? 4 : (d.head == ZEST_HEAD_BLEND ? 5 : 12);
    int dev = 0, cus = 256;
    if (hipGetDevice(&dev) != hipSuccess ||
        hipDeviceGetAttribute(&cus, hipDeviceAttributeMultiprocessorCount, dev) != hipSuccess)
        cus = 256;
    const int n_pass = zest_div_up(zest_div_up(M, 16 * mlp_cb(EP)), kMlpWaves);
    const int blocks = n_pass < cus ? n_pass : cus;
    if ((d.net_type >= 2) != V2) {
        zest_set_error("zest_mlp_fwd(engine): kernel / net_type mismatch");
        return (int)hipErrorInvalidValue;
    }
    hipLaunchKernelGGL((mlp_engine_kernel<EP, NT_PTS, MOD, NT_FEAT, TRAIN, V2>), dim3(blocks), dim3(kMlpWaves * 64), 0, stream,
                       (const uint4 *)tiles, x, M, d.in_ch_pts, F, C_in, C_out, d.head,
                       d.net_type == 2 ? 1 : 0, out, (uint4 *)stash_tiles, (uint2 *)stash_masks);
    ZEST_RETURN_LAUNCH(TRAIN ? "zest_mlp_train16_fwd" : "zest_mlp_fwd(engine)");
}

template <int EP>
static int launch_prec(const MlpPlan &p, const void *tiles, const float *x, int M, float *out, hipStream_t stream) {
    const bool mod = p.desc.use_feat != 0;
    const int key = p.nt_pts * 10 + (mod ? p.nt_feat : 0);
    if (p.desc.net_type >= 2) {
        switch (key) {
            case 42: return launch_one<EP, 4, true, 2, false, true>(p, tiles, x, M, out, stream);
            case 44: return launch_one<EP, 4, true, 4, false, true>(p, tiles, x, M, out, stream);
            case 62: return launch_one<EP, 6, true, 2, false, true>(p, tiles, x, M, out, stream);
            case 64: return launch_one<EP, 6, true, 4, false, true>(p, tiles, x, M, out, stream);
        }
        zest_set_error("zest_mlp_fwd(engine): no 'v2' kernel for %d point units / %d feature units per row block",
                       p.nt_pts, mod ? p.nt_feat : 0);
        return (int)hipErrorInvalidValue;
    }
    switch (key) {
        case 40: return launch_one<EP, 4, false, 0>(p, tiles, x, M, out, stream);
        case 42: return launch_one<EP, 4, true, 2>(p, tiles, x, M, out, stream);
        case 44: return launch_one<EP, 4, true, 4>(p, tiles, x, M, out, stream);
        case 60: return launch_one<EP, 6, false, 0>(p, tiles, x, M, out, stream);
        case 62: return launch_one<EP, 6, true, 2>(p, tiles, x, M, out, stream);
        case 64: return launch_one<EP, 6, true, 4>(p, tiles, x, M, out, stream);
    }
    zest_set_error("zest_mlp_fwd(engine): no kernel for %d point units / %d feature units per row "
                   "block (supported: 1..14 source views)", p.nt_pts, mod ? p.nt_feat : 0);
    return (int)hipErrorInvalidValue;
}

int mlp_engine_train_launch(const MlpPlan &p, const void *tiles, const float *x, int M, float *out, void *stash_tiles,
                            void *stash_masks, hipStream_t stream) {
    constexpr int EP = ZEST_PREC_BF16;
    const bool mod = p.desc.use_feat != 0;
    const int key = p.nt_pts * 10 + (mod ? p.nt_feat : 0);
    switch (key) {
        case 40: return launch_one<EP, 4, false, 0, true>(p, tiles, x, M, out, stream, stash_tiles, stash_masks);
        case 42: return launch_one<EP, 4, true, 2, true>(p, tiles, x, M, out, stream, stash_tiles, stash_masks);
        case 44: return launch_one<EP, 4, true, 4, true>(p, tiles, x, M, out, stream, stash_tiles, stash_masks);
        case 60: return launch_one<EP, 6, false, 0, true>(p, tiles, x, M, out, stream, stash_tiles, stash_masks);
        case 62: return launch_one<EP, 6, true, 2, true>(p, tiles, x, M, out, stream, stash_tiles, stash_masks);
        case 64: return launch_one<EP, 6, true, 4, true>(p, tiles, x, M, out, stream, stash_tiles, stash_masks);
    }
    zest_set_error("zest_mlp_train16_fwd: no kernel for %d point units / %d feature units per row block", p.nt_pts,
                   mod ? p.nt_feat : 0);
    return (int)hipErrorInvalidValue;
}

int mlp_engine_launch(const MlpPlan &p, const void *tiles, const float *x, int M, float *out,
                      hipStream_t stream) {
    switch (p.precision) {
        case ZEST_PREC_BF16: return launch_prec<ZEST_PREC_BF16>(p, tiles, x, M, out, stream);
        case ZEST_PREC_F16: return launch_prec<ZEST_PREC_F16>(p, tiles, x, M, out, stream);
        case ZEST_PREC_F16X3: return launch_prec<ZEST_PREC_F16X3>(p, tiles, x, M, out, stream);
    }
    zest_set_error("zest_mlp_fwd(engine): precision %d is not an engine operand type", p.precision);
    return (int)hipErrorInvalidValue;
}

}
```

### zest-nerf_amd/csrc/mlp_plan.h

```cpp
#pragma once
#include <stdint.h>
#include <vector>
#include "../../include/zest_render.h"

#ifdef __HIPCC__
#define ZEST_HD __host__ __device__
#else
#define ZEST_HD
#endif

namespace zest {

ZEST_HD inline int feat_volume_round(int V) { return V % 4 <= 2 ? V / 4 : V / 4 + 1; }
ZEST_HD inline int feat_quad_col(int q, int V) {
    const int r = 2 * (q >> 3) + (q & 1), g = (q & 7) >> 1, rv = feat_volume_round(V);
    if (r > rv) return -1;
    if (r == rv && g < 2) return 4 * g;
    const int view = r < rv ? 4 * r + g : 4 * rv + g - 2;
    return view < V ? 8 + 4 * view : -1;
}

constexpr int kW = 256;
constexpr int kNumOps = 12;
constexpr int kMaxSeg = 2;
constexpr int kStreamAlign = 128;

constexpr int kFoldSlot = ZEST_P_COUNT;
constexpr int kParamSlots = ZEST_P_COUNT + 1;
constexpr size_t kFoldBiasOffset = (size_t)(kW / 2) * kW * 4;
constexpr size_t kFoldScratchBytes = (kFoldBiasOffset + (size_t)(kW / 2) * 4 + 1023) / 1024 * 1024;
constexpr size_t fold_scratch_offset(size_t plain_bytes) { return plain_bytes; }
constexpr size_t infer_stream_offset(size_t plain_bytes) { return plain_bytes + kFoldScratchBytes; }

enum SlotOrder {
    ORDER_ACC = 0,
    ORDER_NATURAL = 1,
};

enum SegKind { SEG_PTS = 0, SEG_FEAT = 1, SEG_VIEWS = 2, SEG_H = 3 };

struct SegPlan {
    int kind;
    int ntiles;
};

struct OpPlan {
    int njb;
    int nseg;
    SegPlan seg[kMaxSeg];
    int mod;
    int relu;
    int tile_base;
    int tiles_per_jb;
    int bias_block;
};

struct MlpShape {
    int D, W, skip_mask;
    bool is_default;
};
bool mlp_shape(const zest_mlp_desc &d, MlpShape *s, const char **err);
void mlp_param_ld(const zest_mlp_desc &d, const MlpShape &s, int *ld);

struct MlpPlan {
    zest_mlp_desc desc;
    MlpShape shape;
    int n_ops;
    int precision, order;
    int spt;
    int ns_pts, ns_feat, ns_views;
    int nt_pts, nt_feat, nt_views, nt_h, nt_h128;
    int tail_unit0;
    int headers;
    int parts;
    int fold;
    size_t stream_off;
    int n_tiles, n_bias_blocks;
    size_t bias_bytes, bytes;
    OpPlan op[kNumOps];
    std::vector<int16_t> map_pts, map_feat, map_views;
    std::vector<uint32_t> tile_src, bias_src;
    std::vector<uint32_t> hdr_src;
    std::vector<uint8_t> unit_part;
};

inline bool prec_is_engine(int precision) {
    return precision == ZEST_PREC_BF16 || precision == ZEST_PREC_F16 || precision == ZEST_PREC_F16X3;
}

bool build_bwd_plan(const zest_mlp_desc &d, MlpPlan *out, const char **err);
constexpr int bwd_stream_units_raw(int nt_pts, int nt_feat) {
    const int kp = nt_pts / 2, mod = nt_feat;
    return 4 * (1 + 2 * 1)
           + 8 * (1 + 2 * 4)
           + 8 * (1 + mod + 2 * 9)
           + 6 * 8 * (1 + mod + 2 * 8)
           + kp * (1 + 2 * 8) + 8 * (1 + mod + 2 * 8)
           + kp * (1 + 2 * 8);
}
constexpr int bwd_stream_units(int nt_pts, int nt_feat) {
    return (bwd_stream_units_raw(nt_pts, nt_feat) + kStreamAlign - 1) / kStreamAlign * kStreamAlign;
}

struct DwJob {
    int32_t out_tile0, n_out_tiles;
    int32_t in_kind;
    int32_t in_tile0, n_in_tiles;
    int32_t ld, col0, want_bias;
    int32_t wg0, n_wg;
    int16_t out_slot[256], out_row[256];
    int16_t in_col[256];
};
constexpr int kGradTiles = 86;
constexpr int kDwStashPts = 76, kDwStashFeat = 79, kDwStashViews = 81;
int build_dw_jobs(const zest_mlp_desc &d, std::vector<DwJob> *jobs, const char **err);

bool build_plan(const zest_mlp_desc &d, int precision, int order, MlpPlan *out, const char **err,
                bool with_tables = true, bool fold = false);

}
```

### zest-nerf_amd/csrc/mlp_plan.hip

```cpp
#include "mlp_plan.h"
#include <string.h>

namespace zest {

namespace {

inline int round_up(int a, int b) { return (a + b - 1) / b * b; }

void pe_map_acc(int C, int L, int npos, std::vector<int16_t> &m) {
    m.assign((size_t)npos, -1);
    for (int pos = 0; pos < npos; pos++) {
        const int kt = pos / 32, g = (pos % 32) / 8, e = pos % 8, mm = 8 * kt + e;
        if (mm < (L / 2) * C) {
            const int band = 2 * (mm / C) + (g >> 1), coord = mm % C;
            m[pos] = (int16_t)(C + 2 * C * band + ((g & 1) ? C : 0) + coord);
        } else if (mm == (L / 2) * C) {
            m[pos] = (int16_t)(g < C ? g : -1);
        }
    }
}

void feat_map_acc(int V, int npos, std::vector<int16_t> &m) {
    m.assign((size_t)npos, -1);
    for (int pos = 0; pos < npos; pos++) {
        const int kt = pos / 32, g = (pos % 32) / 8, e = pos % 8, q = 8 * kt + 2 * g + (e >> 2), c = e & 3;
        const int col = feat_quad_col(q, V);
        if (col >= 0) m[pos] = (int16_t)(col + c);
    }
}

void natural_map(int width, int spt, int ntiles, std::vector<int16_t> &m) {
    m.assign((size_t)ntiles * spt * 2, -1);
    for (int t = 0; t < ntiles; t++)
        for (int j = 0; j < spt; j++)
            for (int h = 0; h < 2; h++) {
                const int f = t * 2 * spt + spt * h + j;
                m[2 * (t * spt + j) + h] = (int16_t)(f < width ? f : -1);
            }
}

inline int h_feature(int order, int spt, int slot, int half) {
    if (order == ORDER_ACC) {
        const int kt = slot / 32, g = (slot % 32) / 8, e = slot % 8;
        return 32 * kt + (e < 4 ? 4 * g + e : 16 + 4 * g + (e - 4));
    }
    const int t = slot / spt, j = slot % spt;
    return t * 2 * spt + spt * half + j;
}

struct RowSrc { int param, row; };

}

bool build_plan(const zest_mlp_desc &d, int precision, int order, MlpPlan *P, const char **err,
                bool with_tables, bool fold) {
    static const char *e_prec = "precision must be ZEST_PREC_F32, _BF16, _F16 or _F16X3";
    static const char *e_pts = "in_ch_pts must be 63 (xyz, L=10) or 84 (xyzt, L=10)";
    static const char *e_views = "in_ch_views must be 27 (L=4)";
    static const char *e_feat = "in_ch_feat must be 8 + 4V with 1 <= V <= 16 when use_feat is set";
    static const char *e_head = "bad head / net_type combination";
    if (precision != ZEST_PREC_F32 && !prec_is_engine(precision)) return *err = e_prec, false;
    if ((order == ORDER_ACC) != prec_is_engine(precision))
        return *err = "ORDER_ACC goes with the engine precisions, ORDER_NATURAL with fp32", false;
    if (fold && order != ORDER_ACC) return *err = "only the engine's stream (ORDER_ACC) has a folded form", false;
    if (d.in_ch_pts != 63 && d.in_ch_pts != 84) return *err = e_pts, false;
    if (d.in_ch_views != 27) return *err = e_views, false;
    const int F = d.use_feat ? d.in_ch_feat : 0;
    if (d.use_feat && (F < 12 || (F - 8) % 4 != 0 || F > 72)) return *err = e_feat, false;
    if (d.head < 0 || d.head > 2 || (d.net_type != 0 && d.net_type != 2 && d.net_type != 3) ||
        (d.net_type >= 2 && (d.head != 0 || !d.use_feat)))
        return *err = e_head, false;

    MlpShape sh;
    if (!mlp_shape(d, &sh, err)) return false;
    if (order == ORDER_ACC && !sh.is_default)
        return *err = "the MFMA engine covers depth 8 / width 256 / skips [4]; other shapes run in ZEST_PREC_F32", false;
    const int D = sh.D, Wd = sh.W;

    MlpPlan &p = *P;
    p.desc = d, p.precision = precision, p.order = order, p.shape = sh;
    p.n_ops = D + 4;
    p.spt = prec_is_engine(precision) ? 8 : 4;
    p.parts = precision == ZEST_PREC_F16X3 ? 2 : 1;
    p.fold = fold ? 1 : 0, p.stream_off = 0;
    const int spt = p.spt, C = d.in_ch_pts == 63 ? 3 : 4, V = d.use_feat ? (F - 8) / 4 : 0;
    if (order == ORDER_ACC) {
        p.ns_pts = 32 * ((5 * C + 1 + 7) / 8);
        p.ns_views = 32;
        p.ns_feat = d.use_feat ? round_up(4 * (2 + V), 32) : 0;
        pe_map_acc(C, 10, p.ns_pts, p.map_pts);
        pe_map_acc(3, 4, p.ns_views, p.map_views);
        if (d.use_feat) feat_map_acc(V, p.ns_feat, p.map_feat);
    } else {
        p.ns_pts = round_up(d.in_ch_pts, 2 * spt) / 2;
        p.ns_views = round_up(27, 2 * spt) / 2;
        p.ns_feat = d.use_feat ? round_up(F, 2 * spt) / 2 : 0;
        natural_map(d.in_ch_pts, spt, p.ns_pts / spt, p.map_pts);
        natural_map(27, spt, p.ns_views / spt, p.map_views);
        if (d.use_feat) natural_map(F, spt, p.ns_feat / spt, p.map_feat);
    }
    const int spu = order == ORDER_ACC ? 16 : spt;
    p.nt_pts = p.ns_pts / spu, p.nt_views = p.ns_views / spu, p.nt_feat = p.ns_feat / spu;
    p.nt_h = order == ORDER_ACC ? 16 : Wd / 2 / spt, p.nt_h128 = order == ORDER_ACC ? 8 : Wd / 4 / spt;

    p.headers = order == ORDER_ACC ? 1 : 0;
    memset(p.op, 0, sizeof(p.op));
    int tile = 0, bblk = d.use_feat ? Wd / 32 : 0;
    for (int o = 0; o < p.n_ops; o++) {
        OpPlan &op = p.op[o];
        op.njb = Wd / 32, op.nseg = 1, op.seg[0] = {SEG_H, p.nt_h};
        if (o < D) op.mod = d.use_feat ? 1 : 0, op.relu = 1;
        if (o == 0) op.seg[0] = {SEG_PTS, p.nt_pts};
        if (o > 0 && o < D && (sh.skip_mask >> (o - 1) & 1))
            op.nseg = 2, op.seg[0] = {SEG_PTS, p.nt_pts}, op.seg[1] = {SEG_H, p.nt_h};
        if (o == D) op.njb = 1;
        if (o == D + 1 && fold) op.njb = 0;
        if (o == D + 2) op.njb = Wd / 64, op.relu = 1, op.nseg = 2, op.seg[1] = {SEG_VIEWS, p.nt_views};
        if (o == D + 3) op.njb = 1, op.seg[0] = {SEG_H, p.nt_h128};
        op.tiles_per_jb = (op.mod ? p.nt_feat : 0) * p.parts + p.headers;
        for (int s = 0; s < op.nseg; s++) op.tiles_per_jb += op.seg[s].ntiles * p.parts;
        op.tile_base = tile, op.bias_block = bblk;
        tile += op.njb * op.tiles_per_jb, bblk += op.njb;
    }
    if (p.headers) tile = round_up(tile, kStreamAlign), bblk = 0;
    p.n_tiles = tile, p.n_bias_blocks = bblk;
    p.bias_bytes = (size_t)round_up(bblk * 128, 1024);
    p.bytes = p.bias_bytes + (size_t)tile * 1024;
    if (fold) {
        MlpPlan plain;
        if (!build_plan(d, precision, order, &plain, err, false, false)) return false;
        p.stream_off = infer_stream_offset(plain.bytes);
    }

    if (!with_tables) return true;
    int ld[ZEST_P_COUNT];
    mlp_param_ld(d, sh, ld);
    const uint32_t ZERO = 0xFFFFFFFFu;
    p.tile_src.assign((size_t)tile * 64 * spt, ZERO);
    p.bias_src.assign(p.bias_bytes / 4, ZERO);
    p.hdr_src.assign(p.headers ? (size_t)tile * 64 : 0, ZERO);
    p.unit_part.assign((size_t)tile, 0);

    auto row_src = [&](int o, int row) -> RowSrc {
        if (o < D) return {ZEST_P_PTS0 + o, row};
        if (o == D + 1) return {ZEST_P_FEATURE, row};
        if (o == D + 2) return {row < Wd / 2 ? (fold ? kFoldSlot : ZEST_P_VIEWS) : -1, row};
        if (o == D + 3) return {row < 3 ? ZEST_P_RGB : -1, row};
        if (row == 0) return {ZEST_P_ALPHA, 0};
        if (d.head == ZEST_HEAD_BLEND && row == 1) return {ZEST_P_HEAD0, 0};
        if (d.head == ZEST_HEAD_DYNAMIC && row >= 1 && row <= 6) return {ZEST_P_HEAD0, row - 1};
        if (d.head == ZEST_HEAD_DYNAMIC && row >= 7 && row <= 8) return {ZEST_P_HEAD1, row - 7};
        return {-1, 0};
    };
    auto emit_tiles = [&](int &t, int param_of_rows_op, int jb, const SegPlan &sg, int col0,
                          bool is_mod) {
        for (int k = 0; k < sg.ntiles; k++)
          for (int part = 0; part < p.parts; part++, t++) {
            p.unit_part[t] = (uint8_t)part;
            for (int l = 0; l < 64; l++)
                for (int e = 0; e < spt; e++) {
                    int slot, half, row, feat;
                    if (order == ORDER_ACC) {
                        slot = (k / 2) * 32 + 8 * (l >> 4) + e, half = 0, row = 32 * jb + 16 * (k % 2) + (l & 15);
                        switch (sg.kind) {
                            case SEG_PTS: feat = p.map_pts[slot]; break;
                            case SEG_FEAT: feat = p.map_feat[slot]; break;
                            case SEG_VIEWS: feat = p.map_views[slot]; break;
                            default: feat = h_feature(order, spt, slot, 0);
                        }
                    } else {
                        slot = k * spt + e, half = l >> 5, row = 32 * jb + (l & 31);
                        switch (sg.kind) {
                            case SEG_PTS: feat = p.map_pts[2 * slot + half]; break;
                            case SEG_FEAT: feat = p.map_feat[2 * slot + half]; break;
                            case SEG_VIEWS: feat = p.map_views[2 * slot + half]; break;
                            default: feat = h_feature(order, spt, slot, half);
                        }
                    }
                    RowSrc rs = is_mod ? RowSrc{ZEST_P_PTS_BIAS, row} : row_src(param_of_rows_op, row);
                    if (feat < 0 || rs.param < 0) continue;
                    const bool folded_h = rs.param == kFoldSlot && sg.kind == SEG_H;
                    const int param = rs.param == kFoldSlot && !folded_h ? (int)ZEST_P_VIEWS : rs.param;
                    const int ldp = folded_h ? Wd : ld[param];
                    p.tile_src[((size_t)t * 64 + l) * spt + e] =
                        ((uint32_t)param << 24) | (uint32_t)(rs.row * ldp + col0 + feat);
                }
          }
    };
    auto emit_bias_to = [&](std::vector<uint32_t> &dst, size_t at, int o, int jb, bool is_mod) {
        for (int h = 0; h < 2; h++)
            for (int i = 0; i < 16; i++) {
                const int row = order == ORDER_ACC ? 32 * jb + 16 * h + i
                                                   : 32 * jb + (i & 3) + 8 * (i >> 2) + 4 * h;
                RowSrc rs = is_mod ? RowSrc{ZEST_P_PTS_BIAS, row} : row_src(o, row);
                if (rs.param < 0) continue;
                dst[at + h * 16 + i] = ((uint32_t)rs.param << 24) | rs.row;
            }
    };
    auto emit_bias = [&](int block, int o, int jb, bool is_mod) {
        emit_bias_to(p.bias_src, (size_t)block * 32, o, jb, is_mod);
    };
    if (d.use_feat && !p.headers)
        for (int jb = 0; jb < Wd / 32; jb++) emit_bias(jb, 0, jb, true);
    for (int o = 0; o < p.n_ops; o++) {
        const OpPlan &op = p.op[o];
        int t = op.tile_base;
        for (int jb = 0; jb < op.njb; jb++) {
            if (p.headers) {
                emit_bias_to(p.hdr_src, (size_t)t * 64, o, jb, false);
                if (op.mod) emit_bias_to(p.hdr_src, (size_t)t * 64 + 32, o, jb, true);
                t++;
            } else {
                emit_bias(op.bias_block + jb, o, jb, false);
            }
            if (op.mod) emit_tiles(t, o, jb, SegPlan{SEG_FEAT, p.nt_feat}, 0, true);
            int col0 = 0;
            for (int s = 0; s < op.nseg; s++) {
                emit_tiles(t, o, jb, op.seg[s], col0, false);
                col0 += op.seg[s].kind == SEG_PTS ? d.in_ch_pts : Wd;
            }
        }
    }
    return true;
}

bool mlp_shape(const zest_mlp_desc &d, MlpShape *s, const char **err) {
    const bool unset = d.depth == 0 && d.width == 0 && d.skip_mask == 0;
    s->D = unset ? 8 : d.depth, s->W = unset ? kW : d.width, s->skip_mask = unset ? 1 << 4 : d.skip_mask;
    if (s->D < 2 || s->D > 8) return *err = "depth must be 2 .. 8", false;
    if (s->W != 64 && s->W != 128 && s->W != 192 && s->W != 256) return *err = "width must be 64, 128, 192 or 256", false;
    if (s->skip_mask < 0 || (s->skip_mask >> (s->D - 1)) != 0) return *err = "skip_mask names a layer beyond depth", false;
    s->is_default = s->D == 8 && s->W == kW && s->skip_mask == 1 << 4;
    return true;
}

void mlp_param_ld(const zest_mlp_desc &d, const MlpShape &s, int *ld) {
    for (int l = 0; l < 8; l++)
        ld[ZEST_P_PTS0 + l] = l == 0 ? d.in_ch_pts : s.W + ((s.skip_mask >> (l - 1) & 1) ? d.in_ch_pts : 0);
    ld[ZEST_P_PTS_BIAS] = d.in_ch_feat, ld[ZEST_P_VIEWS] = s.W + d.in_ch_views, ld[ZEST_P_FEATURE] = s.W;
    ld[ZEST_P_ALPHA] = s.W, ld[ZEST_P_RGB] = s.W / 2, ld[ZEST_P_HEAD0] = s.W, ld[ZEST_P_HEAD1] = s.W;
}


namespace {

struct BwdCtx {
    const zest_mlp_desc &d;
    MlpPlan &p;
    int ld[ZEST_P_COUNT];
    int t = 0;
    std::vector<uint32_t> tile_src, hdr_src;
    void grow(int units) {
        tile_src.resize((size_t)(t + units) * 512, 0xFFFFFFFFu);
        hdr_src.resize((size_t)(t + units) * 64, 0xFFFFFFFFu);
    }
};

inline RowSrc out_row_of(const zest_mlp_desc &d, int op, int o) {
    if (op == 100) return {ZEST_P_PTS_BIAS, o};
    if (op < 8) return {ZEST_P_PTS0 + op, o};
    if (op == 9) return {ZEST_P_FEATURE, o};
    if (op == 10) return {o < kW / 2 ? ZEST_P_VIEWS : -1, o};
    if (op == 11) return {o < 3 ? ZEST_P_RGB : -1, o};
    if (o == 0) return {ZEST_P_ALPHA, 0};
    if (d.head == ZEST_HEAD_BLEND && o == 1) return {ZEST_P_HEAD0, 0};
    if (d.head == ZEST_HEAD_DYNAMIC && o >= 1 && o <= 6) return {ZEST_P_HEAD0, o - 1};
    if (d.head == ZEST_HEAD_DYNAMIC && o >= 7 && o <= 8) return {ZEST_P_HEAD1, o - 7};
    return {-1, 0};
}

template <class InCol>
void emit_bwd_row_block(BwdCtx &c, InCol in_col, int mod_jb, const int (*segs)[2], int nseg) {
    const MlpPlan &p = c.p;
    int units = 1 + (mod_jb >= 0 ? p.nt_feat : 0);
    for (int s = 0; s < nseg; s++) units += 2 * segs[s][1];
    c.grow(units);
    if (mod_jb >= 0)
        for (int i = 0; i < 32; i++)
            c.hdr_src[(size_t)c.t * 64 + 32 + i] = ((uint32_t)ZEST_P_PTS_BIAS << 24) | (uint32_t)(32 * mod_jb + i);
    c.t++;
    if (mod_jb >= 0)
        for (int k = 0; k < p.nt_feat; k++, c.t++)
            for (int l = 0; l < 64; l++)
                for (int e = 0; e < 8; e++) {
                    const int pos = (k / 2) * 32 + 8 * (l >> 4) + e, row = 32 * mod_jb + 16 * (k % 2) + (l & 15);
                    const int feat = p.map_feat[pos];
                    if (feat < 0) continue;
                    c.tile_src[((size_t)c.t * 64 + l) * 8 + e] =
                        ((uint32_t)ZEST_P_PTS_BIAS << 24) | (uint32_t)(row * c.ld[ZEST_P_PTS_BIAS] + feat);
                }
    for (int s = 0; s < nseg; s++)
        for (int k = 0; k < 2 * segs[s][1]; k++, c.t++)
            for (int l = 0; l < 64; l++)
                for (int e = 0; e < 8; e++) {
                    const int pos = (k / 2) * 32 + 8 * (l >> 4) + e;
                    const int o = h_feature(ORDER_ACC, 8, pos, 0);
                    const RowSrc rs = out_row_of(c.d, segs[s][0], o);
                    const int col = in_col(16 * (k % 2) + (l & 15));
                    if (rs.param < 0 || col < 0) continue;
                    c.tile_src[((size_t)c.t * 64 + l) * 8 + e] =
                        ((uint32_t)rs.param << 24) | (uint32_t)(rs.row * c.ld[rs.param] + col);
                }
}

}

bool build_bwd_plan(const zest_mlp_desc &d, MlpPlan *P, const char **err) {
    if (!build_plan(d, ZEST_PREC_BF16, ORDER_ACC, P, err, false)) return false;
    if (d.net_type != 0) return *err = "the bf16 training path covers 'v0' nets", false;
    MlpPlan &p = *P;
    BwdCtx c{d, p, {d.in_ch_pts, kW, kW, kW, kW, kW + d.in_ch_pts, kW, kW, d.in_ch_feat, kW + d.in_ch_views, kW, kW,
                    kW / 2, kW, kW}};
    const bool mod = d.use_feat != 0;
    const int kp = p.nt_pts / 2;
    auto natural = [](int base) { return [base](int i) { return base + i; }; };
    for (int jb = 0; jb < 4; jb++) { const int sg[1][2] = {{11, 1}}; emit_bwd_row_block(c, natural(32 * jb), -1, sg, 1); }
    for (int jb = 0; jb < 8; jb++) { const int sg[1][2] = {{10, 4}}; emit_bwd_row_block(c, natural(32 * jb), -1, sg, 1); }
    for (int jb = 0; jb < 8; jb++) { const int sg[2][2] = {{9, 8}, {8, 1}}; emit_bwd_row_block(c, natural(32 * jb), mod ? jb : -1, sg, 2); }
    for (int l = 7; l >= 1; l--) {
        const int sg[1][2] = {{l, 8}};
        if (l == 5)
            for (int jb = 0; jb < kp; jb++)
                emit_bwd_row_block(c, [&](int i) { return (int)p.map_pts[32 * jb + i]; }, -1, sg, 1);
        const int h0 = l == 5 ? d.in_ch_pts : 0;
        for (int jb = 0; jb < 8; jb++) emit_bwd_row_block(c, natural(h0 + 32 * jb), mod ? jb : -1, sg, 1);
    }
    for (int jb = 0; jb < kp; jb++) {
        const int sg[1][2] = {{0, 8}};
        emit_bwd_row_block(c, [&](int i) { return (int)p.map_pts[32 * jb + i]; }, -1, sg, 1);
    }
    if (c.t != bwd_stream_units_raw(p.nt_pts, mod ? p.nt_feat : 0)) return *err = "backward stream: unit count mismatch", false;
    int total = round_up(c.t, kStreamAlign);
    c.grow(total - c.t);
    c.t = total;
    p.tail_unit0 = total;
    if (mod) {
        for (int jb = 0; jb < p.nt_feat / 2; jb++) {
            const int sg[1][2] = {{100, 8}};
            emit_bwd_row_block(c, [&](int i) { return (int)p.map_feat[32 * jb + i]; }, -1, sg, 1);
        }
        for (int jb = 0; jb < 8; jb++) emit_bwd_row_block(c, [](int) { return -1; }, jb, nullptr, 0);
    }
    total = c.t;
    p.headers = 1, p.parts = 1, p.n_tiles = total, p.n_bias_blocks = 0, p.bias_bytes = 0;
    p.bytes = (size_t)total * 1024;
    p.tile_src.swap(c.tile_src), p.hdr_src.swap(c.hdr_src);
    p.bias_src.clear();
    p.unit_part.assign((size_t)total, 0);
    return true;
}

int build_dw_jobs(const zest_mlp_desc &d, std::vector<DwJob> *jobs, const char **err) {
    MlpPlan p;
    if (!build_plan(d, ZEST_PREC_BF16, ORDER_ACC, &p, err, false)) return -1;
    jobs->clear();
    const bool mod = d.use_feat != 0;
    const int kp = p.nt_pts / 2, kf = p.nt_feat / 2;
    auto add = [&](int op, int out_tile0, int n_out, int in_kind, int in_tile0, int n_in, int ld, int col0, int bias,
                   const std::vector<int16_t> *in_map) {
        DwJob j;
        memset(&j, 0, sizeof(j));
        j.out_tile0 = out_tile0, j.n_out_tiles = n_out, j.in_kind = in_kind, j.in_tile0 = in_tile0, j.n_in_tiles = n_in;
        j.ld = ld, j.col0 = col0, j.want_bias = bias;
        for (int pos = 0; pos < 256; pos++) {
            j.out_slot[pos] = -1, j.out_row[pos] = 0, j.in_col[pos] = -1;
            if (pos < 32 * n_out) {
                const int o = h_feature(ORDER_ACC, 8, pos, 0);
                const RowSrc rs = out_row_of(d, op, o);
                j.out_slot[pos] = (int16_t)rs.param, j.out_row[pos] = (int16_t)rs.row;
            }
            if (pos < 32 * n_in)
                j.in_col[pos] = in_map ? (*in_map)[pos] : (int16_t)h_feature(ORDER_ACC, 8, pos, 0);
        }
        jobs->push_back(j);
    };
    for (int l = 0; l < 8; l++) {
        const int ld = l == 0 ? d.in_ch_pts : (l == 5 ? kW + d.in_ch_pts : kW);
        if (l == 0 || l == 5) add(l, 8 * l, 8, 1, kDwStashPts, kp, ld, 0, l == 0, &p.map_pts);
        if (l > 0) add(l, 8 * l, 8, 0, 8 * (l - 1), 8, ld, l == 5 ? d.in_ch_pts : 0, 1, nullptr);
    }
    add(8, 76, 1, 0, 56, 8, kW, 0, 1, nullptr);
    add(9, 64, 8, 0, 56, 8, kW, 0, 1, nullptr);
    add(10, 72, 4, 0, 64, 8, kW + d.in_ch_views, 0, 1, nullptr);
    add(10, 72, 4, 3, kDwStashViews, 1, kW + d.in_ch_views, kW, 0, &p.map_views);
    add(11, 77, 1, 0, 72, 4, kW / 2, 0, 1, nullptr);
    if (mod) add(100, 78, 8, 2, kDwStashFeat, kf, d.in_ch_feat, 0, 1, &p.map_feat);
    return (int)jobs->size();
}

}
```

Measured before the change: 10.93 million rays/s.

## Compact inference weight stream: bias table in LDS, drop header units and unused row tiles

Adds a compact form of the folded inference weight stream. Per-row-block bias headers are moved out of the streamed ring into a bias table staged once in LDS at kernel start. Half the tiles of the alpha and final ops, which only need row tile 0, are dropped, and the ring uses 6 slots sized for the new tile count. The goal is fewer bytes streamed from global memory per pass and fewer ring units to wait on. The cost is extra LDS for the table, an upfront staging load with a full vmcnt wait, and more complex plan and packing logic.

```diff
diff --git a/zest-nerf_amd/csrc/fused.cuh b/zest-nerf_amd/csrc/fused.cuh
--- a/zest-nerf_amd/csrc/fused.cuh
+++ b/zest-nerf_amd/csrc/fused.cuh
@@ -283,19 +283,22 @@
     constexpr bool MOD_S = NT_FEAT_S > 0, MOD_D = NT_FEAT_D > 0;
     constexpr int NP = ep_parts(EP), CB = fused_cb(EP), BS = 16 * CB;
     if constexpr (EP == ZEST_PREC_F16) engine_fp16_overflow_clamp();
-    constexpr int UNITS_S = stream_units(4, NT_FEAT_S, NP, true), UNITS_D = DYN ? stream_units(6, NT_FEAT_D, NP, true) : 0;
-    using Ring = RingTiles<kFusedWaves, UNITS_S, UNITS_D>;
+    constexpr InferLayout LAY_S = infer_layout(4, NT_FEAT_S, NP), LAY_D = infer_layout(6, NT_FEAT_D, NP);
+    constexpr int UNITS_S = LAY_S.units, UNITS_D = DYN ? LAY_D.units : 0;
+    using Ring = RingTiles<kFusedWaves, UNITS_S, UNITS_D, kInferSlots, false, LAY_S.bias_stride, DYN ? LAY_D.bias_stride : 0>;
+    constexpr int kRingBytes = Ring::kRingUnits * 1024;
+    constexpr int kWeightBytes = kRingBytes + Ring::kTableBytes > kRingUnits * 1024 ? kRingBytes + Ring::kTableBytes : kRingUnits * 1024;
     constexpr bool FEATURELESS = !MOD_S && !MOD_D;
     constexpr int PF = (NP == 1 && FEATURELESS) ? kPrefetchLone : kPrefetch;
     constexpr bool CONT = NP == 1 || FEATURELESS;
     constexpr int kStBytes = DYN ? kFusedWaves * 32 * 24 : 0;
     constexpr int kGapBytes = 2 * kSlots * 4;
-    __shared__ __attribute__((aligned(16))) char lds[kRingUnits * 1024 + 2 * kMaxViews * kCamStride * 4 +
+    __shared__ __attribute__((aligned(16))) char lds[kWeightBytes + 2 * kMaxViews * kCamStride * 4 +
                                                      kFusedWaves * 32 * 8 + kGapBytes +
                                                      kFusedWaves * kPartialFloats * 4 + kFusedWaves * 32 * 16 +
                                                      kStBytes + 2 * kCarryFloats * 4];
     static_assert(sizeof(lds) <= 163840, "LDS budget of one workgroup per CU");
-    float *cams_s = reinterpret_cast<float *>(lds + kRingUnits * 1024), *cams_d = cams_s + kMaxViews * kCamStride;
+    float *cams_s = reinterpret_cast<float *>(lds + kWeightBytes), *cams_d = cams_s + kMaxViews * kCamStride;
     float2 *zd_lds = reinterpret_cast<float2 *>(cams_d + kMaxViews * kCamStride);
     constexpr bool PROJ = EP != ZEST_PREC_F16X3;
     stage_cams<PROJ>(a.st, cams_s);
@@ -305,14 +308,15 @@
     float4 *x_lds = reinterpret_cast<float4 *>(rec_lds + kFusedWaves * kPartialFloats);
     float2 *st_lds = reinterpret_cast<float2 *>(x_lds + kFusedWaves * 32);
     float *carry_lds = reinterpret_cast<float *>(reinterpret_cast<char *>(st_lds) + kStBytes);
-    __syncthreads();
-
     const int lane0 = threadIdx.x & 63;
     const int wave = __builtin_amdgcn_readfirstlane(threadIdx.x >> 6);
     const Ring tiles{lds, (gptr_u4)a.st.tiles, (gptr_u4)a.dy.tiles, lane0, lane0 >> 4, wave,
                      (unsigned)(wave * Ring::kPieces * 64 + lane0) * 16u,
                      (unsigned)(uintptr_t)(__attribute__((address_space(3))) char *)lds +
                          (unsigned)wave * Ring::kPieces * 1024u};
+    tiles.stage_bias_table(lds + kRingBytes, (int)threadIdx.x);
+    __syncthreads();
+
     tiles.init_addr();
     tiles.prologue();
 
@@ -543,7 +547,7 @@
         ZEST_RETURN_LAUNCH("zest_render_fused_fwd(" #ptag "_" #tag ")");                         \
     }                                                                                            \
     int fused_units_##ptag##_##tag(int which) {                                                  \
-        return which == 0 ? stream_units(4, NTS, ep_parts(EP), true) : (DYN ? stream_units(6, NTD, ep_parts(EP), true) : 0); \
+        return which == 0 ? infer_layout(4, NTS, ep_parts(EP)).units : (DYN ? infer_layout(6, NTD, ep_parts(EP)).units : 0); \
     }
 
 #define ZEST_FUSED_DECL1(ptag, tag)                                                     \
diff --git a/zest-nerf_amd/csrc/fused.hip b/zest-nerf_amd/csrc/fused.hip
--- a/zest-nerf_amd/csrc/fused.hip
+++ b/zest-nerf_amd/csrc/fused.hip
@@ -23,12 +23,12 @@
     if (d->in_ch_pts != pts_ch) return *err = "unexpected in_ch_pts for this slot", false;
     if (d->net_type != 0 && d->net_type != 2) return *err = "net_type must be 0 ('v0') or 2 ('v2')", false;
     zest::MlpPlan plan;
-    if (!zest::build_plan(*d, precision, zest::ORDER_ACC, &plan, err, false, true)) return false;
+    if (!zest::build_plan(*d, precision, zest::ORDER_ACC, &plan, err, false, true, true)) return false;
     n->bias = (const float *)((const char *)packed + plan.stream_off);
     n->tiles = (const uint4 *)((const char *)n->bias + plan.bias_bytes);
     n->head = d->head, n->v2 = d->net_type == 2;
     *nt_feat = d->use_feat ? plan.nt_feat : 0;
-    *units = plan.n_tiles;
+    *units = plan.ring_units;
     if (((uintptr_t)packed & 15) != 0) return *err = "packed weights must be 16-byte aligned", false;
     if (vs) {
         n->w2cs = vs->w2cs, n->intr = vs->intrinsics;
diff --git a/zest-nerf_amd/csrc/mlp.hip b/zest-nerf_amd/csrc/mlp.hip
--- a/zest-nerf_amd/csrc/mlp.hip
+++ b/zest-nerf_amd/csrc/mlp.hip
@@ -34,7 +34,7 @@
         dp = new DevPlan();
         const char *err = nullptr;
         const bool ok = order == kOrderBwd    ? zest::build_bwd_plan(d, &dp->plan, &err)
-                        : order == kOrderFold ? zest::build_plan(d, precision, zest::ORDER_ACC, &dp->plan, &err, true, true)
+                        : order == kOrderFold ? zest::build_plan(d, precision, zest::ORDER_ACC, &dp->plan, &err, true, true, true)
                                               : zest::build_plan(d, precision, order, &dp->plan, &err);
         if (!ok) {
             zest_set_error("MLP shape not supported: %s", err);
@@ -117,13 +117,13 @@
 }
 
 __global__ void pack_headers_kernel(ParamTable pt, const uint32_t *__restrict__ hdr_src, size_t n,
-                                    char *__restrict__ w_out) {
+                                    char *__restrict__ w_out, int per, int pitch) {
     const size_t i = (size_t)blockIdx.x * blockDim.x + threadIdx.x;
     if (i >= n) return;
     const uint32_t s = hdr_src[i];
     if (s == 0xFFFFFFFFu) return;
-    const size_t unit = i / 64, j = i % 64;
-    ((float *)(w_out + unit * 1024))[j] = pt.p[2 * (s >> 24) + 1][s & 0xFFFFFF];
+    const size_t block = i / per, j = i % per;
+    ((float *)(w_out + block * pitch))[j] = pt.p[2 * (s >> 24) + 1][s & 0xFFFFFF];
 }
 
 struct F32Op {
@@ -272,7 +272,7 @@
     hipLaunchKernelGGL(pack_kernel<ZEST_PREC_BF16>, dim3(zest_div_up(n_w, 256)), dim3(256), 0, stream, pt, dp->tile_src,
                        n_w, dp->bias_src, (size_t)0, dp->unit_part, (float *)packed, packed);
     hipLaunchKernelGGL(pack_headers_kernel, dim3(zest_div_up(n_h, 256)), dim3(256), 0, stream, pt, dp->hdr_src, n_h,
-                       (char *)packed);
+                       (char *)packed, 64, 1024);
     ZEST_RETURN_LAUNCH("zest_mlp_train16_pack");
 }
 }
@@ -319,9 +319,12 @@
             else if (precision == ZEST_PREC_F16) ZEST_PACK(ZEST_PREC_F16);
             else ZEST_PACK(ZEST_PREC_F16X3);
             const size_t n_h = q->plan.hdr_src.size();
+            const bool table = q->plan.compact != 0;
             if (n_h)
                 hipLaunchKernelGGL(pack_headers_kernel, dim3(zest_div_up(n_h, 256)), dim3(256), 0,
-                                   (hipStream_t)stream, pt, q->hdr_src, n_h, (char *)w_out);
+                                   (hipStream_t)stream, pt, q->hdr_src, n_h,
+                                   (char *)w_out + (table ? (size_t)q->plan.ring_units * 1024 : 0),
+                                   table ? q->plan.bias_stride / 4 : 64, table ? q->plan.bias_stride : 1024);
         } else {
             ZEST_PACK(ZEST_PREC_F32);
         }
diff --git a/zest-nerf_amd/csrc/mlp_engine.cuh b/zest-nerf_amd/csrc/mlp_engine.cuh
--- a/zest-nerf_amd/csrc/mlp_engine.cuh
+++ b/zest-nerf_amd/csrc/mlp_engine.cuh
@@ -12,14 +12,6 @@
 
 namespace zest {
 
-constexpr int stream_units_raw(int nt_pts, int nt_feat, int parts = 1, bool fold = false) {
-    const int mod = nt_feat * parts, P = nt_pts * parts, H = 16 * parts;
-    return 8 * (1 + mod + P) + 6 * 8 * (1 + mod + H) + 8 * (1 + mod + P + H)
-           + (1 + H) + (fold ? 0 : 8 * (1 + H)) + 4 * (1 + H + 2 * parts) + (1 + H / 2);
-}
-constexpr int stream_units(int nt_pts, int nt_feat, int parts = 1, bool fold = false) {
-    return (stream_units_raw(nt_pts, nt_feat, parts, fold) + kStreamAlign - 1) / kStreamAlign * kStreamAlign;
-}
 static_assert(stream_units_raw(4, 0) == 1262 && stream_units_raw(4, 0, 1, true) == 1126 &&
               stream_units(4, 0, 1, true) == 9 * kStreamAlign, "unit counts of the headline net (DESIGN.md 3.1)");
 
@@ -35,8 +27,16 @@
 #ifndef ZEST_ISSUERS
 #define ZEST_ISSUERS 8
 #endif
-template <int NW, int UNITS_A, int UNITS_B>
+template <int NW, int UNITS_A, int UNITS_B, int SLOTS = kSlots, bool HEADERS = true, int BIAS_A = 0, int BIAS_B = 0,
+          int AHEAD = kAhead>
 struct RingTiles {
+    static constexpr int kSlots = SLOTS, kRingUnits = kChunk * SLOTS, kAhead = AHEAD;
+    static constexpr bool kHeaders = HEADERS;
+    static constexpr int kHeader = HEADERS ? 1 : 0;
+    static constexpr int kKeepRowTiles = HEADERS ? 2 : 1;
+    static constexpr int kTableBytesA = kInferBlocks * BIAS_A, kTableBytes = kInferBlocks * (BIAS_A + BIAS_B);
+    static_assert(kSlots >= kAhead + 1, "a slot is refilled while the previous chunk may still be read");
+    static_assert(HEADERS || kTableBytes <= 65536, "the bias table is read with one base register and the DS offset field");
     static constexpr int kIssuers = ZEST_ISSUERS < NW ? ZEST_ISSUERS : NW;
     static constexpr int kPieces = kChunk / kIssuers;
     static constexpr int kChunksA = UNITS_A / kChunk, kChunks = (UNITS_A + UNITS_B) / kChunk;
@@ -116,9 +116,33 @@
         return *reinterpret_cast<const bf16x8 *>(&v);
     }
     __device__ __forceinline__ f32x4 load_bias(int unit, int which, int rt) const {
+        static_assert(HEADERS, "a header unit is read");
         if (which == 0 && rt == 0) touch(unit);
         const int r = unit % kRingUnits;
         return *lds_at<v4f>((r < 64 ? rb_lo : rb_hi) + (r % 64) * 1024 + which * 128 + rt * 64);
+    }
+    mutable unsigned tb = 0;
+    __device__ __forceinline__ f32x4 load_bias(int unit, int block, int which, int rt) const {
+        if constexpr (HEADERS) {
+            return load_bias(unit, which, rt);
+        } else {
+            const bool net_a = unit % (UNITS_A + UNITS_B) < UNITS_A;
+            return *lds_at<v4f>(tb + (net_a ? block * BIAS_A : kTableBytesA + block * BIAS_B) + which * 128 + rt * 64);
+        }
+    }
+    __device__ __forceinline__ void stage_bias_table(char *table_lds, int tid) const {
+        static_assert(!HEADERS, "header-form streams carry their biases");
+        const unsigned base = (unsigned)(uintptr_t)(__attribute__((address_space(3))) char *)table_lds;
+        tb = base + grp * 16;
+        asm volatile("" : "+v"(tb));
+        uint4 *dst = reinterpret_cast<uint4 *>(table_lds);
+        const uint4 *ta = (const uint4 *)src_a + (size_t)UNITS_A * 64;
+        for (int i = tid; i < kTableBytesA / 16; i += NW * 64) dst[i] = ta[i];
+        if (UNITS_B > 0) {
+            const uint4 *tbl = (const uint4 *)src_b + (size_t)UNITS_B * 64;
+            for (int i = tid; i < (kTableBytes - kTableBytesA) / 16; i += NW * 64) dst[kTableBytesA / 16 + i] = tbl[i];
+        }
+        asm volatile("s_waitcnt vmcnt(0)" ::: "memory");
     }
     __device__ __forceinline__ void finish(int unit, int end) const {
 #pragma unroll
@@ -224,7 +248,7 @@
 
 template <int EP, int CB, int NJB, int NKA, int NKB, bool MOD, int NKF, bool RELU, int MODE, bool V2, int PF, bool CONT,
           class Tiles, class Sink = NoSink>
-__device__ __forceinline__ void engine_layer(const Tiles &tiles, int &unit,
+__device__ __forceinline__ void engine_layer(const Tiles &tiles, int &unit, int &block,
                                              const OpArr<NKA, ep_parts(EP)> (&opa)[CB],
                                              const OpArr<NKB, ep_parts(EP)> (&opb)[CB],
                                              const OpArr<NKF, ep_parts(EP)> (&opf)[CB],
@@ -232,28 +256,30 @@
                                              int sink_id = 0, const Sink &sink = Sink()) {
     constexpr int NP = ep_parts(EP);
     constexpr bool X3 = EP == ZEST_PREC_F16X3;
-    constexpr int NM = MOD ? 2 * NKF : 0, T = NM + 2 * (NKA + NKB);
+    constexpr int HDR = Tiles::kHeader, RT = MODE == 1 ? Tiles::kKeepRowTiles : 2;
+    constexpr int NM = MOD ? 2 * NKF : 0, T = NM + RT * (NKA + NKB);
     static_assert(T >= 1, "empty layer");
+    static_assert(RT == 2 || !MOD, "an op that keeps row tile 0 only is not modulated");
     constexpr bool kPackedRelu = RELU && MODE == 0 && EP != ZEST_PREC_F16X3 && __is_same(Sink, NoSink);
     constexpr int P = PF < T ? PF : T;
-    auto preload_header = [&](RowBlockPre<NP, PF> &p, int u0) {
+    auto preload_header = [&](RowBlockPre<NP, PF> &p, int u0, int jb) {
 #pragma unroll
         for (int rt = 0; rt < 2; rt++) {
-            p.bias[rt] = tiles.load_bias(u0, 0, rt);
-            if (MOD) p.mbias[rt] = tiles.load_bias(u0, 1, rt);
+            p.bias[rt] = tiles.load_bias(u0, block + jb, 0, rt);
+            if (MOD) p.mbias[rt] = tiles.load_bias(u0, block + jb, 1, rt);
         }
     };
     auto preload_tile = [&](RowBlockPre<NP, PF> &p, int u0, int k) {
 #pragma unroll
-        for (int pt = 0; pt < NP; pt++) p.win[k][pt] = tiles.load(u0 + 1 + NP * k + pt);
+        for (int pt = 0; pt < NP; pt++) p.win[k][pt] = tiles.load(u0 + HDR + NP * k + pt);
     };
-    auto preload = [&](RowBlockPre<NP, PF> &p, int u0) {
-        preload_header(p, u0);
+    auto preload = [&](RowBlockPre<NP, PF> &p, int u0, int jb) {
+        preload_header(p, u0, jb);
 #pragma unroll
         for (int k = 0; k < P; k++) preload_tile(p, u0, k);
     };
     RowBlockPre<NP, PF> pre;
-    preload(pre, unit);
+    preload(pre, unit, 0);
 #pragma unroll
     for (int jb = 0; jb < NJB; jb++) {
         const int u0 = unit;
@@ -276,7 +302,7 @@
             bf16x8 a[NP];
 #pragma unroll
             for (int pt = 0; pt < NP; pt++) a[pt] = win[k % P][pt];
-            const int rt = k % 2, kt = (k < NM ? k : k - NM) / 2;
+            const int rt = k < NM ? k % 2 : (k - NM) % RT, kt = k < NM ? k / 2 : (k - NM) / RT;
 #pragma unroll
             for (int cb = 0; cb < CB; cb++) {
                 auto opnd = [&](int pt) -> bf16x8 {
@@ -300,14 +326,14 @@
             }
             if (k + P < T) {
 #pragma unroll
-                for (int pt = 0; pt < NP; pt++) win[k % P][pt] = tiles.load(u0 + 1 + NP * (k + P) + pt);
+                for (int pt = 0; pt < NP; pt++) win[k % P][pt] = tiles.load(u0 + HDR + NP * (k + P) + pt);
             } else if (CONT && jb + 1 < NJB) {
-                if (k + P == T) preload_header(pre, u0 + 1 + NP * T);
-                preload_tile(pre, u0 + 1 + NP * T, k + P - T);
+                if (k + P == T) preload_header(pre, u0 + HDR + NP * T, jb + 1);
+                preload_tile(pre, u0 + HDR + NP * T, k + P - T);
             }
         }
-        unit = u0 + 1 + NP * T;
-        if (!CONT && jb + 1 < NJB) preload(pre, unit);
+        unit = u0 + HDR + NP * T;
+        if (!CONT && jb + 1 < NJB) preload(pre, unit, jb + 1);
 #pragma unroll
         for (int cb = 0; cb < CB; cb++) {
             float v[8];
@@ -339,6 +365,7 @@
             }
         }
     }
+    block += NJB;
 }
 
 template <int EP, int CB, int NU_PTS, bool MOD, int NU_FEAT, bool V2, bool FOLD = false, int PF = kPrefetch,
@@ -352,29 +379,31 @@
     OpArr<0, NP> none[CB];
     f32x4 unused[CB];
     const int unit0 = unit;
+    int block = 0;
+    static_assert(Tiles::kHeaders || FOLD, "the compact stream is the inference stream");
     {
         OpArr<KP, NP> pts[CB];
         pts_fn(pts);
-        engine_layer<EP, CB, 8, KP, 0, MOD, KF, true, 0, V2, PF, CONT>(tiles, unit, pts, none, feat, hA, unused, 0, sink);
-    }
-    engine_layer<EP, CB, 8, 8, 0, MOD, KF, true, 0, V2, PF, CONT>(tiles, unit, hA, none, feat, hB, unused, 1, sink);
-    engine_layer<EP, CB, 8, 8, 0, MOD, KF, true, 0, V2, PF, CONT>(tiles, unit, hB, none, feat, hA, unused, 2, sink);
-    engine_layer<EP, CB, 8, 8, 0, MOD, KF, true, 0, V2, PF, CONT>(tiles, unit, hA, none, feat, hB, unused, 3, sink);
-    engine_layer<EP, CB, 8, 8, 0, MOD, KF, true, 0, V2, PF, CONT>(tiles, unit, hB, none, feat, hA, unused, 4, sink);
+        engine_layer<EP, CB, 8, KP, 0, MOD, KF, true, 0, V2, PF, CONT>(tiles, unit, block, pts, none, feat, hA, unused, 0, sink);
+    }
+    engine_layer<EP, CB, 8, 8, 0, MOD, KF, true, 0, V2, PF, CONT>(tiles, unit, block, hA, none, feat, hB, unused, 1, sink);
+    engine_layer<EP, CB, 8, 8, 0, MOD, KF, true, 0, V2, PF, CONT>(tiles, unit, block, hB, none, feat, hA, unused, 2, sink);
+    engine_layer<EP, CB, 8, 8, 0, MOD, KF, true, 0, V2, PF, CONT>(tiles, unit, block, hA, none, feat, hB, unused, 3, sink);
+    engine_layer<EP, CB, 8, 8, 0, MOD, KF, true, 0, V2, PF, CONT>(tiles, unit, block, hB, none, feat, hA, unused, 4, sink);
     {
         OpArr<KP, NP> pts[CB];
         pts_fn(pts);
-        engine_layer<EP, CB, 8, KP, 8, MOD, KF, true, 0, V2, PF, CONT>(tiles, unit, pts, hA, feat, hB, unused, 5, sink);
-    }
-    engine_layer<EP, CB, 8, 8, 0, MOD, KF, true, 0, V2, PF, CONT>(tiles, unit, hB, none, feat, hA, unused, 6, sink);
-    engine_layer<EP, CB, 8, 8, 0, MOD, KF, true, 0, V2, PF, CONT>(tiles, unit, hA, none, feat, hB, unused, 7, sink);
-    engine_layer<EP, CB, 1, 8, 0, false, KF, false, 1, V2, PF, CONT>(tiles, unit, hB, none, feat, hA, head);
+        engine_layer<EP, CB, 8, KP, 8, MOD, KF, true, 0, V2, PF, CONT>(tiles, unit, block, pts, hA, feat, hB, unused, 5, sink);
+    }
+    engine_layer<EP, CB, 8, 8, 0, MOD, KF, true, 0, V2, PF, CONT>(tiles, unit, block, hB, none, feat, hA, unused, 6, sink);
+    engine_layer<EP, CB, 8, 8, 0, MOD, KF, true, 0, V2, PF, CONT>(tiles, unit, block, hA, none, feat, hB, unused, 7, sink);
+    engine_layer<EP, CB, 1, 8, 0, false, KF, false, 1, V2, PF, CONT>(tiles, unit, block, hB, none, feat, hA, head);
     if constexpr (!FOLD)
-        engine_layer<EP, CB, 8, 8, 0, false, KF, false, 0, V2, PF, CONT>(tiles, unit, hB, none, feat, hA, unused, 8, sink);
+        engine_layer<EP, CB, 8, 8, 0, false, KF, false, 0, V2, PF, CONT>(tiles, unit, block, hB, none, feat, hA, unused, 8, sink);
     OpArr<8, NP> (&vin)[CB] = FOLD ? hB : hA, (&vout)[CB] = FOLD ? hA : hB;
     OpArr<1, NP> views[CB];
     views_fn(views);
-    engine_layer<EP, CB, 4, 8, 1, false, KF, true, 0, V2, PF, CONT>(tiles, unit, vin, views, feat, vout, unused, 9, sink);
+    engine_layer<EP, CB, 4, 8, 1, false, KF, true, 0, V2, PF, CONT>(tiles, unit, block, vin, views, feat, vout, unused, 9, sink);
     OpArr<4, NP> h128[CB];
 #pragma unroll
     for (int cb = 0; cb < CB; cb++)
@@ -382,9 +411,11 @@
         for (int pt = 0; pt < NP; pt++)
 #pragma unroll
             for (int k = 0; k < 4; k++) h128[cb].t[pt][k] = vout[cb].t[pt][k];
-    engine_layer<EP, CB, 1, 4, 0, false, KF, false, 1, V2, PF, CONT>(tiles, unit, h128, none, feat, vin, rgb);
-    tiles.finish(unit, unit0 + stream_units(NU_PTS, MOD ? NU_FEAT : 0, NP, FOLD));
-    unit = unit0 + stream_units(NU_PTS, MOD ? NU_FEAT : 0, NP, FOLD);
+    engine_layer<EP, CB, 1, 4, 0, false, KF, false, 1, V2, PF, CONT>(tiles, unit, block, h128, none, feat, vin, rgb);
+    constexpr int UNITS = Tiles::kHeaders ? stream_units(NU_PTS, MOD ? NU_FEAT : 0, NP, FOLD)
+                                          : infer_layout(NU_PTS, MOD ? NU_FEAT : 0, NP).units;
+    tiles.finish(unit, unit0 + UNITS);
+    unit = unit0 + UNITS;
 }
 
 int mlp_engine_launch(const MlpPlan &p, const void *tiles, const float *x, int M, float *out,
diff --git a/zest-nerf_amd/csrc/mlp_engine.hip b/zest-nerf_amd/csrc/mlp_engine.hip
--- a/zest-nerf_amd/csrc/mlp_engine.hip
+++ b/zest-nerf_amd/csrc/mlp_engine.hip
@@ -1,3 +1,4 @@
+#include <type_traits>
 #include "mlp_engine.cuh"
 #include "mlp_train16.h"
 #include "mlp_operands.cuh"
@@ -39,16 +40,23 @@
     const uint4 *__restrict__ tiles_g, const float *__restrict__ x, int M, int P, int F, int C_in, int C_out, int head,
     int act_out, float *__restrict__ out, uint4 *__restrict__ stash_tiles = nullptr, uint2 *__restrict__ stash_masks = nullptr) {
     constexpr bool FOLD = !TRAIN;
-    constexpr int NP = ep_parts(EP), CB = mlp_cb(EP), UNITS = stream_units(NT_PTS, MOD ? NT_FEAT : 0, NP, FOLD);
-    using Ring = RingTiles<kMlpWaves, UNITS, 0>;
+    constexpr InferLayout LAY = infer_layout(NT_PTS, MOD ? NT_FEAT : 0, ep_parts(EP));
+    constexpr int NP = ep_parts(EP), CB = mlp_cb(EP), UNITS = FOLD ? LAY.units : stream_units(NT_PTS, MOD ? NT_FEAT : 0, NP, false);
+    using Ring = std::conditional_t<FOLD, RingTiles<kMlpWaves, UNITS, 0, kInferSlots, false, LAY.bias_stride>,
+                                    RingTiles<kMlpWaves, UNITS, 0>>;
     if constexpr (EP == ZEST_PREC_F16) engine_fp16_overflow_clamp();
     __shared__ __attribute__((aligned(16))) char lds[kRingUnits * 1024 + 2 * kSlots * 4];
+    static_assert(Ring::kRingUnits * 1024 + Ring::kTableBytes <= kRingUnits * 1024, "ring and bias table");
     const int lane = threadIdx.x & 63, col = lane & 15, grp = lane >> 4;
     const int wave = __builtin_amdgcn_readfirstlane(threadIdx.x >> 6);
     const Ring tiles{lds, (gptr_u4)tiles_g, (gptr_u4)tiles_g, lane, grp, wave,
                      (unsigned)(wave * Ring::kPieces * 64 + lane) * 16u,
                      (unsigned)(uintptr_t)(__attribute__((address_space(3))) char *)lds +
                          (unsigned)wave * Ring::kPieces * 1024u};
+    if constexpr (FOLD) {
+        tiles.stage_bias_table(lds + Ring::kRingUnits * 1024, (int)threadIdx.x);
+        __syncthreads();
+    }
     tiles.init_addr();
     tiles.prologue();
     const int n_blocks = (M + 16 * CB - 1) / (16 * CB), n_pass = (n_blocks + kMlpWaves - 1) / kMlpWaves;
@@ -123,9 +131,10 @@
 template <int EP, int NT_PTS, bool MOD, int NT_FEAT, bool TRAIN = false, bool V2 = false>
 static int launch_one(const MlpPlan &p, const void *tiles, const float *x, int M,
                       float *out, hipStream_t stream, void *stash_tiles = nullptr, void *stash_masks = nullptr) {
-    constexpr int units = stream_units(NT_PTS, MOD ? NT_FEAT : 0, ep_parts(EP), !TRAIN);
-    if (p.n_tiles != units || (p.fold != 0) != !TRAIN) {
-        zest_set_error("zest_mlp_fwd(engine): plan has %d stream units (fold %d), kernel expects %d (fold %d)", p.n_tiles,
+    constexpr int units = TRAIN ? stream_units(NT_PTS, MOD ? NT_FEAT : 0, ep_parts(EP), false)
+                                : infer_layout(NT_PTS, MOD ? NT_FEAT : 0, ep_parts(EP)).units;
+    if (p.ring_units != units || (p.fold != 0) != !TRAIN || (p.compact != 0) != !TRAIN) {
+        zest_set_error("zest_mlp_fwd(engine): plan has %d stream units (fold %d), kernel expects %d (fold %d)", p.ring_units,
                        p.fold, units, TRAIN ? 0 : 1);
         return (int)hipErrorInvalidValue;
     }
diff --git a/zest-nerf_amd/csrc/mlp_plan.h b/zest-nerf_amd/csrc/mlp_plan.h
--- a/zest-nerf_amd/csrc/mlp_plan.h
+++ b/zest-nerf_amd/csrc/mlp_plan.h
@@ -31,6 +31,43 @@
 constexpr size_t kFoldScratchBytes = (kFoldBiasOffset + (size_t)(kW / 2) * 4 + 1023) / 1024 * 1024;
 constexpr size_t fold_scratch_offset(size_t plain_bytes) { return plain_bytes; }
 constexpr size_t infer_stream_offset(size_t plain_bytes) { return plain_bytes + kFoldScratchBytes; }
+
+constexpr int stream_units_raw(int nt_pts, int nt_feat, int parts = 1, bool fold = false) {
+    const int mod = nt_feat * parts, P = nt_pts * parts, H = 16 * parts;
+    return 8 * (1 + mod + P) + 6 * 8 * (1 + mod + H) + 8 * (1 + mod + P + H)
+           + (1 + H) + (fold ? 0 : 8 * (1 + H)) + 4 * (1 + H + 2 * parts) + (1 + H / 2);
+}
+constexpr int stream_units(int nt_pts, int nt_feat, int parts = 1, bool fold = false) {
+    return (stream_units_raw(nt_pts, nt_feat, parts, fold) + kStreamAlign - 1) / kStreamAlign * kStreamAlign;
+}
+
+constexpr int kInferSlots = 6, kInferRing = kInferSlots * 16;
+constexpr int kInferBlocks = 8 * 8 + 1 + 4 + 1;
+struct InferLayout {
+    int tiles;
+    int units;
+    int bias_stride;
+    int table_bytes;
+    int region;
+};
+constexpr InferLayout infer_layout(int nt_pts, int nt_feat, int parts = 1) {
+    const int H = 16 * parts;
+    const int tiles = stream_units_raw(nt_pts, nt_feat, parts, true) - kInferBlocks - H / 2 - H / 4;
+    const int stride = nt_feat ? 256 : 128;
+    return InferLayout{tiles, (tiles + kInferRing - 1) / kInferRing * kInferRing, stride, kInferBlocks * stride,
+                       stream_units(nt_pts, nt_feat, parts, true)};
+}
+constexpr bool infer_layout_fits(int nt_pts, int nt_feat, int parts) {
+    const InferLayout l = infer_layout(nt_pts, nt_feat, parts);
+    return l.units % kInferRing == 0 && (size_t)l.units * 1024 + (size_t)l.table_bytes <= (size_t)l.region * 1024;
+}
+static_assert(infer_layout_fits(4, 0, 1) && infer_layout_fits(4, 2, 1) && infer_layout_fits(4, 4, 1) &&
+              infer_layout_fits(6, 0, 1) && infer_layout_fits(6, 2, 1) && infer_layout_fits(6, 4, 1) &&
+              infer_layout_fits(4, 0, 2) && infer_layout_fits(4, 2, 2) && infer_layout_fits(4, 4, 2) &&
+              infer_layout_fits(6, 0, 2) && infer_layout_fits(6, 2, 2) && infer_layout_fits(6, 4, 2),
+              "padded tiles + bias table fit the inference region of every shape the engine supports");
+static_assert(infer_layout(4, 0).units == 1056 && infer_layout(4, 0).table_bytes == 8960 && infer_layout(4, 0).region == 1152,
+              "the headline net: 66 chunks per pass");
 
 enum SlotOrder {
     ORDER_ACC = 0,
@@ -75,6 +112,9 @@
     int parts;
     int fold;
     size_t stream_off;
+    int compact;
+    int ring_units;
+    int bias_stride;
     int n_tiles, n_bias_blocks;
     size_t bias_bytes, bytes;
     OpPlan op[kNumOps];
@@ -116,6 +156,6 @@
 int build_dw_jobs(const zest_mlp_desc &d, std::vector<DwJob> *jobs, const char **err);
 
 bool build_plan(const zest_mlp_desc &d, int precision, int order, MlpPlan *out, const char **err,
-                bool with_tables = true, bool fold = false);
+                bool with_tables = true, bool fold = false, bool compact = false);
 
 }
diff --git a/zest-nerf_amd/csrc/mlp_plan.hip b/zest-nerf_amd/csrc/mlp_plan.hip
--- a/zest-nerf_amd/csrc/mlp_plan.hip
+++ b/zest-nerf_amd/csrc/mlp_plan.hip
@@ -53,7 +53,7 @@
 }
 
 bool build_plan(const zest_mlp_desc &d, int precision, int order, MlpPlan *P, const char **err,
-                bool with_tables, bool fold) {
+                bool with_tables, bool fold, bool compact) {
     static const char *e_prec = "precision must be ZEST_PREC_F32, _BF16, _F16 or _F16X3";
     static const char *e_pts = "in_ch_pts must be 63 (xyz, L=10) or 84 (xyzt, L=10)";
     static const char *e_views = "in_ch_views must be 27 (L=4)";
@@ -63,6 +63,7 @@
     if ((order == ORDER_ACC) != prec_is_engine(precision))
         return *err = "ORDER_ACC goes with the engine precisions, ORDER_NATURAL with fp32", false;
     if (fold && order != ORDER_ACC) return *err = "only the engine's stream (ORDER_ACC) has a folded form", false;
+    if (compact && !fold) return *err = "only the inference stream (fold) has a compact form", false;
     if (d.in_ch_pts != 63 && d.in_ch_pts != 84) return *err = e_pts, false;
     if (d.in_ch_views != 27) return *err = e_views, false;
     const int F = d.use_feat ? d.in_ch_feat : 0;
@@ -82,7 +83,7 @@
     p.n_ops = D + 4;
     p.spt = prec_is_engine(precision) ? 8 : 4;
     p.parts = precision == ZEST_PREC_F16X3 ? 2 : 1;
-    p.fold = fold ? 1 : 0, p.stream_off = 0;
+    p.fold = fold ? 1 : 0, p.stream_off = 0, p.compact = compact ? 1 : 0, p.bias_stride = 0;
     const int spt = p.spt, C = d.in_ch_pts == 63 ? 3 : 4, V = d.use_feat ? (F - 8) / 4 : 0;
     if (order == ORDER_ACC) {
         p.ns_pts = 32 * ((5 * C + 1 + 7) / 8);
@@ -103,9 +104,11 @@
     p.nt_pts = p.ns_pts / spu, p.nt_views = p.ns_views / spu, p.nt_feat = p.ns_feat / spu;
     p.nt_h = order == ORDER_ACC ? 16 : Wd / 2 / spt, p.nt_h128 = order == ORDER_ACC ? 8 : Wd / 4 / spt;
 
-    p.headers = order == ORDER_ACC ? 1 : 0;
+    p.headers = order == ORDER_ACC && !compact ? 1 : 0;
     memset(p.op, 0, sizeof(p.op));
     int tile = 0, bblk = d.use_feat ? Wd / 32 : 0;
+    int region = 0;
+    auto rt0_only = [&](int o) { return compact && (o == D || o == D + 3); };
     for (int o = 0; o < p.n_ops; o++) {
         OpPlan &op = p.op[o];
         op.njb = Wd / 32, op.nseg = 1, op.seg[0] = {SEG_H, p.nt_h};
@@ -118,11 +121,25 @@
         if (o == D + 2) op.njb = Wd / 64, op.relu = 1, op.nseg = 2, op.seg[1] = {SEG_VIEWS, p.nt_views};
         if (o == D + 3) op.njb = 1, op.seg[0] = {SEG_H, p.nt_h128};
         op.tiles_per_jb = (op.mod ? p.nt_feat : 0) * p.parts + p.headers;
-        for (int s = 0; s < op.nseg; s++) op.tiles_per_jb += op.seg[s].ntiles * p.parts;
+        int full = op.tiles_per_jb + (compact ? 1 : 0);
+        for (int s = 0; s < op.nseg; s++) {
+            op.tiles_per_jb += op.seg[s].ntiles / (rt0_only(o) ? 2 : 1) * p.parts;
+            full += op.seg[s].ntiles * p.parts;
+        }
         op.tile_base = tile, op.bias_block = bblk;
-        tile += op.njb * op.tiles_per_jb, bblk += op.njb;
-    }
-    if (p.headers) tile = round_up(tile, kStreamAlign), bblk = 0;
+        tile += op.njb * op.tiles_per_jb, bblk += op.njb, region += op.njb * full;
+    }
+    p.ring_units = tile;
+    if (p.headers) tile = round_up(tile, kStreamAlign), bblk = 0, p.ring_units = tile;
+    if (compact) {
+        const InferLayout lay = infer_layout(p.nt_pts, d.use_feat ? p.nt_feat : 0, p.parts);
+        if (tile != lay.tiles || bblk - (d.use_feat ? Wd / 32 : 0) != kInferBlocks || round_up(region, kStreamAlign) != lay.region)
+            return *err = "compact inference stream: unit count mismatch", false;
+        if (!infer_layout_fits(p.nt_pts, d.use_feat ? p.nt_feat : 0, p.parts))
+            return *err = "compact inference stream: tiles and bias table do not fit the inference region", false;
+        p.ring_units = lay.units, p.bias_stride = lay.bias_stride;
+        tile = lay.region, bblk = 0;
+    }
     p.n_tiles = tile, p.n_bias_blocks = bblk;
     p.bias_bytes = (size_t)round_up(bblk * 128, 1024);
     p.bytes = p.bias_bytes + (size_t)tile * 1024;
@@ -138,7 +155,7 @@
     const uint32_t ZERO = 0xFFFFFFFFu;
     p.tile_src.assign((size_t)tile * 64 * spt, ZERO);
     p.bias_src.assign(p.bias_bytes / 4, ZERO);
-    p.hdr_src.assign(p.headers ? (size_t)tile * 64 : 0, ZERO);
+    p.hdr_src.assign(p.headers ? (size_t)tile * 64 : compact ? (size_t)kInferBlocks * p.bias_stride / 4 : 0, ZERO);
     p.unit_part.assign((size_t)tile, 0);
 
     auto row_src = [&](int o, int row) -> RowSrc {
@@ -152,10 +169,12 @@
         if (d.head == ZEST_HEAD_DYNAMIC && row >= 7 && row <= 8) return {ZEST_P_HEAD1, row - 7};
         return {-1, 0};
     };
-    auto emit_tiles = [&](int &t, int param_of_rows_op, int jb, const SegPlan &sg, int col0,
+    auto emit_tiles = [&](int &next, int param_of_rows_op, int jb, const SegPlan &sg, int col0,
                           bool is_mod) {
         for (int k = 0; k < sg.ntiles; k++)
-          for (int part = 0; part < p.parts; part++, t++) {
+          for (int part = 0; part < p.parts; part++) {
+            if (!is_mod && k % 2 == 1 && rt0_only(param_of_rows_op)) continue;
+            const int t = next++;
             p.unit_part[t] = (uint8_t)part;
             for (int l = 0; l < 64; l++)
                 for (int e = 0; e < spt; e++) {
@@ -200,13 +219,18 @@
     auto emit_bias = [&](int block, int o, int jb, bool is_mod) {
         emit_bias_to(p.bias_src, (size_t)block * 32, o, jb, is_mod);
     };
-    if (d.use_feat && !p.headers)
+    if (d.use_feat && !p.headers && !compact)
         for (int jb = 0; jb < Wd / 32; jb++) emit_bias(jb, 0, jb, true);
+    int table_block = 0;
     for (int o = 0; o < p.n_ops; o++) {
         const OpPlan &op = p.op[o];
         int t = op.tile_base;
         for (int jb = 0; jb < op.njb; jb++) {
-            if (p.headers) {
+            if (compact) {
+                const size_t at = (size_t)table_block++ * p.bias_stride / 4;
+                emit_bias_to(p.hdr_src, at, o, jb, false);
+                if (op.mod) emit_bias_to(p.hdr_src, at + 32, o, jb, true);
+            } else if (p.headers) {
                 emit_bias_to(p.hdr_src, (size_t)t * 64, o, jb, false);
                 if (op.mod) emit_bias_to(p.hdr_src, (size_t)t * 64 + 32, o, jb, true);
                 t++;
```

Result: no change. 10.98 million rays/s, median of 6 (+0.5%).
